# big-nacho/patolette

Measured on AMD Instinct MI355X. Metric: Mpixels/sec quantized (256-color ICtCp + KMeans) at 1 GPU; palette ΔE vs ref, higher is better.
Workload: dtype f64

## Files before the change

patolette_amd/csrc/devutil.h:

```cpp
#pragma once

#include <hip/hip_runtime.h>
#include <stdint.h>

namespace pamd {

constexpr int kWave = 64;

struct BinK {
    double M0, M1;
};

__host__ __device__ inline BinK make_bink(int E, int P) {
    int B = 51 - P;
    if (B > 40) B = 40;
    if (B < 8) B = 8;
    BinK k;
    k.M0 = ldexp(1.5, 52 + E - B);
    k.M1 = ldexp(1.5, 52 + E - 2 * B);
    return k;
}

__device__ __forceinline__ void bin_add(double v, const BinK k, double &a0, double &a1) {
    double v0 = (v + k.M0) - k.M0;
    double r = v - v0;
    double v1 = (r + k.M1) - k.M1;
    a0 += v0;
    a1 += v1;
}
__device__ __forceinline__ void bin_split(double v, const BinK k, double &v0, double &v1) {
    v0 = (v + k.M0) - k.M0;
    double r = v - v0;
    v1 = (r + k.M1) - k.M1;
}

__device__ __forceinline__ double wave_sum(double v) {
#pragma unroll
    for (int o = 32; o > 0; o >>= 1) v += __shfl_down(v, o, 64);
    return v;
}
template <int CTRL, int ROW_MASK>
__device__ __forceinline__ double dpp_add_f64(const double v) {
    const int lo = __double2loint(v), hi = __double2hiint(v);
    const int tlo = __builtin_amdgcn_update_dpp(0, lo, CTRL, ROW_MASK, 0xf, true);
    const int thi = __builtin_amdgcn_update_dpp(0, hi, CTRL, ROW_MASK, 0xf, true);
    return v + __hiloint2double(thi, tlo);
}
__device__ __forceinline__ double wave_sum_dpp63(double v) {
    v = dpp_add_f64<0x111, 0xf>(v);
    v = dpp_add_f64<0x112, 0xf>(v);
    v = dpp_add_f64<0x114, 0xf>(v);
    v = dpp_add_f64<0x118, 0xf>(v);
    v = dpp_add_f64<0x142, 0xa>(v);
    v = dpp_add_f64<0x143, 0xc>(v);
    return v;
}
__device__ __forceinline__ unsigned wave_sum_u32(unsigned v) {
#pragma unroll
    for (int o = 32; o > 0; o >>= 1) v += __shfl_down(v, o, 64);
    return v;
}

__device__ __forceinline__ unsigned wave_scan_incl_u32(unsigned v) {
    v += (unsigned)__builtin_amdgcn_update_dpp(0, (int)v, 0x111, 0xf, 0xf, true);
    v += (unsigned)__builtin_amdgcn_update_dpp(0, (int)v, 0x112, 0xf, 0xf, true);
    v += (unsigned)__builtin_amdgcn_update_dpp(0, (int)v, 0x114, 0xf, 0xf, true);
    v += (unsigned)__builtin_amdgcn_update_dpp(0, (int)v, 0x118, 0xf, 0xf, true);
    v += (unsigned)__builtin_amdgcn_update_dpp(0, (int)v, 0x142, 0xa, 0xf, true);
    v += (unsigned)__builtin_amdgcn_update_dpp(0, (int)v, 0x143, 0xc, 0xf, true);
    return v;
}

template <int NV>
__device__ __forceinline__ void block_sum(double (&v)[NV], double *smem) {
    const int lane = threadIdx.x & 63, wid = threadIdx.x >> 6, nw = blockDim.x >> 6;
#pragma unroll
    for (int i = 0; i < NV; i++) v[i] = wave_sum(v[i]);
    if (lane == 0) {
#pragma unroll
        for (int i = 0; i < NV; i++) smem[wid * NV + i] = v[i];
    }
    __syncthreads();
    if (threadIdx.x == 0) {
        for (int w = 1; w < nw; w++) {
#pragma unroll
            for (int i = 0; i < NV; i++) v[i] += smem[w * NV + i];
        }
    }
    __syncthreads();
}

__host__ __device__ inline unsigned long long f64_key(double d) {
    union { double f; unsigned long long u; } c;
    c.f = d;
    return (c.u & 0x8000000000000000ULL) ? ~c.u : (c.u | 0x8000000000000000ULL);
}
__host__ __device__ inline double key_f64(unsigned long long k) {
    union { double f; unsigned long long u; } c;
    c.u = (k & 0x8000000000000000ULL) ? (k & 0x7FFFFFFFFFFFFFFFULL) : ~k;
    return c.f;
}

__host__ __device__ inline unsigned long long splitmix64(unsigned long long x) {
    x += 0x9E3779B97F4A7C15ULL;
    unsigned long long z = x;
    z = (z ^ (z >> 30)) * 0xBF58476D1CE4E5B9ULL;
    z = (z ^ (z >> 27)) * 0x94D049BB133111EBULL;
    return z ^ (z >> 31);
}
__host__ __device__ inline double u01(unsigned long long seed, unsigned long long i) {
    return (double)(splitmix64((seed << 32) + i) >> 11) * 0x1.0p-53;
}

}
```

patolette_amd/csrc/pipeline.hip:

```cpp
#include <algorithm>
#include <functional>
#include <chrono>
#include <cmath>
#include <atomic>
#include <memory>
#include <mutex>
#include <thread>
#include <future>

#include "color_device.h"
#include "common.h"
#include "host_math.h"
#include "kmeans.h"
#include "map.h"
#include "saliency.h"
#include "quant.h"
#include "rgba.h"
#include "compact.h"

namespace pamd {

void launch_convert(int which, const double *src, double *dst, size_t n, ConvertStats *stats, hipStream_t s, BinK sumk = BinK{0.0, 0.0},
                    BinK momk = BinK{0.0, 0.0}, size_t begin = 0, size_t end = ~(size_t)0, bool init_stats = true);
void launch_convert_rows(int which, const double *rows, double *dst, size_t n, ConvertStats *stats, hipStream_t s,
                         BinK sumk = BinK{0.0, 0.0}, BinK momk = BinK{0.0, 0.0}, size_t begin = 0, size_t end = ~(size_t)0,
                         bool init_stats = true);
void launch_convert_u8(int which, const unsigned char *pixels, int channels, double *dst, size_t n, ConvertStats *stats,
                       hipStream_t s, BinK sumk = BinK{0.0, 0.0}, BinK momk = BinK{0.0, 0.0}, size_t begin = 0, size_t end = ~(size_t)0,
                       bool init_stats = true);
void launch_reconstruct(const void *map, int map_elem, size_t n, const unsigned char *pal_u8, int k, unsigned char *out,
                        hipStream_t s);
void launch_weight_stats(const double *w, size_t n, ConvertStats *stats, hipStream_t s);
void launch_pow(const double *x, double y, double *out, size_t n, hipStream_t s);
void launch_fill_image(double *d, size_t n, uint64_t seed, hipStream_t s);
void launch_fill_weights(double *d, size_t n, uint64_t seed, hipStream_t s);

KernelTimer &ktimer() { static thread_local KernelTimer *t = new KernelTimer; return *t; }

std::atomic<int> g_debug_ws{getenv("PAMD_DEBUG_WORKSPACE") ? atoi(getenv("PAMD_DEBUG_WORKSPACE")) & (kWsPoison | kWsCount | kWsLog) : 0};
std::atomic<unsigned long long> g_late_growths{0};
WsStreams &ws_streams() { static thread_local WsStreams w; return w; }
void ws_growth(size_t bytes, const char *file, int line) {
    const int dbg = g_debug_ws.load(std::memory_order_relaxed);
    if (!(dbg & (kWsCount | kWsLog))) return;
    bool queued = false;
    for (const hipStream_t *sp : ws_streams().s)
        if (sp && *sp && hipStreamQuery(*sp) == hipErrorNotReady) queued = true;
    if (!queued) return;
    g_late_growths.fetch_add(1);
    if (dbg & kWsLog) fprintf(stderr, "patolette_amd: workspace growth to %zu bytes while work is queued (%s:%d)\n", bytes, file, line);
}
void ws_poison_dev(void *p, size_t bytes) {
    if (!bytes) return;
    HIP_CHECK(hipMemsetAsync(p, 0xFF, bytes, nullptr));
    HIP_CHECK(hipStreamSynchronize(nullptr));
}
void ws_poison_dev_rows(void *p, size_t pitch, size_t width, size_t rows) {
    if (!width || !rows) return;
    HIP_CHECK(hipMemset2DAsync(p, pitch, 0xFF, width, rows, nullptr));
    HIP_CHECK(hipStreamSynchronize(nullptr));
}
int KernelTimer::id_of(const char *name) {
    for (size_t i = 0; i < names.size(); i++) if (names[i] == name) return (int)i;
    names.emplace_back(name); total_ms.push_back(0); total_bytes.push_back(0); launches.push_back(0);
    return (int)names.size() - 1;
}
hipEvent_t KernelTimer::get_event() {
    if (!pool.empty()) { hipEvent_t e = pool.back(); pool.pop_back(); return e; }
    hipEvent_t e; HIP_CHECK(hipEventCreate(&e)); return e;
}
void KernelTimer::begin(int id, hipStream_t s, double bytes, const double *src) {
    Rec r; r.id = id; r.bytes = bytes; r.src = src; r.a = get_event(); r.b = get_event();
    HIP_CHECK(hipEventRecord(r.a, s));
    pending.push_back(r);
}
void KernelTimer::end(hipStream_t s) { HIP_CHECK(hipEventRecord(pending.back().b, s)); }
void KernelTimer::collect() {
    for (auto &r : pending) {
        float ms = 0;
        if (hipEventSynchronize(r.b) == hipSuccess && hipEventElapsedTime(&ms, r.a, r.b) == hipSuccess && !(r.src && *r.src == 0.0)) {
            total_ms[r.id] += ms; total_bytes[r.id] += r.src ? r.bytes * *r.src : r.bytes; launches[r.id] += 1;
        }
        pool.push_back(r.a); pool.push_back(r.b);
    }
    pending.clear();
}
void KernelTimer::reset() { collect(); names.clear(); total_ms.clear(); total_bytes.clear(); launches.clear(); }

__global__ __launch_bounds__(256) void k_gq_prepare(Tile *tA, int ntA, Tile *tP, int ntP, unsigned long long N, int *round_nodes, int *node_tile0,
                                                    double *hist, unsigned long long nhist, unsigned long long *hsize, unsigned int *hcount) {
    const unsigned long long stride = (unsigned long long)gridDim.x * blockDim.x, t0 = (unsigned long long)blockIdx.x * blockDim.x + threadIdx.x;
    for (unsigned long long i = t0; i < (unsigned long long)ntA; i += stride) {
        const unsigned long long o = i * (unsigned long long)kTileA;
        tA[i] = Tile{o, (unsigned)(N - o < (unsigned long long)kTileA ? N - o : (unsigned long long)kTileA), 0u};
    }
    for (unsigned long long i = t0; i < (unsigned long long)ntP; i += stride) {
        const unsigned long long o = i * (unsigned long long)kTileP;
        tP[i] = Tile{o, (unsigned)(N - o < (unsigned long long)kTileP ? N - o : (unsigned long long)kTileP), 0u};
    }
    for (unsigned long long i = t0; i < nhist; i += stride) hist[i] = 0.0;
    for (unsigned long long i = t0; i < (unsigned long long)kBuckets; i += stride) { hsize[i] = 0ULL; hcount[i] = 0u; }
    if (t0 == 0) { round_nodes[0] = 0; node_tile0[0] = 0; node_tile0[1] = ntP; }
}

__global__ void k_put_nodes(NodeDev *table, const NodeIn *stage, const int *ids, int n) {
    int i = blockIdx.x * blockDim.x + threadIdx.x;
    if (i >= n) return;
    const NodeIn in = stage[i];
    NodeDev &d = table[ids[i]];
    d.begin = in.begin; d.n = in.n; d.gn = in.gn; d.buf = in.buf; d.slot = in.slot; d.child0 = in.child0; d.nchild = in.nchild;
    for (int j = 0; j < 3; j++) { d.axis[j] = in.axis[j]; d.mean[j] = in.mean[j]; }
    d.sw = in.sw; d.klin = in.klin; d.kquad = in.kquad;
    node_reset_outputs(d);
    d.split = in.split; d.psplit = -1;
}
__global__ void k_put_node1(NodeDev *table, const int id, const NodeIn in) {
    NodeDev &d = table[id];
    d.begin = in.begin; d.n = in.n; d.gn = in.gn; d.buf = in.buf; d.slot = in.slot; d.child0 = in.child0; d.nchild = in.nchild;
    for (int j = 0; j < 3; j++) { d.axis[j] = in.axis[j]; d.mean[j] = in.mean[j]; }
    d.sw = in.sw; d.klin = in.klin; d.kquad = in.kquad;
    node_reset_outputs(d);
    d.split = in.split; d.psplit = -1;
}
__global__ void k_get_nodes(const NodeDev *table, NodeOut *stage, const int *ids, int n) {
    int i = blockIdx.x * blockDim.x + threadIdx.x;
    if (i >= n) return;
    const NodeDev &d = table[ids[i]];
    NodeOut o;
    o.begin = d.begin; o.n = d.n; o.gn = d.gn; o.buf = d.buf; o.degenerate = d.degenerate; o.split = d.split; o.psplit = d.psplit;
    o.sw = d.sw;
    for (int j = 0; j < 3; j++) o.mean[j] = d.mean[j];
    for (int q = 0; q < 7; q++) {
        double s0 = 0, s1 = 0;
        for (int k = 0; k < kSlots; k++) { s0 += d.acc[k][q][0]; s1 += d.acc[k][q][1]; }
        o.acc[q][0] = s0; o.acc[q][1] = s1;
    }
    stage[i] = o;
}

struct RoundSetup {
    const NodeIn *recs; const int *ids; const int *tA0; const int *tP0;
    int nr, ntA, ntP;
    Tile *tilesA, *tilesP;
    double *hist; size_t nhist;
    unsigned long long *hsize; unsigned int *hcount; size_t nbk;
};
__device__ __forceinline__ int node_of_tile(const int *t0, int nr, int t) {
    int lo = 0, hi = nr;
    while (hi - lo > 1) { const int mid = (lo + hi) >> 1; if (t0[mid] <= t) lo = mid; else hi = mid; }
    return lo;
}
__global__ __launch_bounds__(256) void k_round_setup(NodeDev *table, RoundSetup a) {
    const size_t tid = (size_t)blockIdx.x * blockDim.x + threadIdx.x, stride = (size_t)gridDim.x * blockDim.x;
    for (size_t i = tid; i < (size_t)a.nr; i += stride) {
        const NodeIn in = a.recs[i];
        NodeDev &d = table[a.ids[i]];
        d.begin = in.begin; d.n = in.n; d.gn = in.gn; d.buf = in.buf; d.slot = in.slot; d.child0 = in.child0; d.nchild = in.nchild;
        for (int j = 0; j < 3; j++) { d.axis[j] = in.axis[j]; d.mean[j] = in.mean[j]; }
        d.sw = in.sw; d.klin = in.klin; d.kquad = in.kquad;
    }
    for (size_t i = tid; i < (size_t)a.nr * kNodeResetElems; i += stride)
        node_reset_element(table[a.ids[i / kNodeResetElems]], (int)(i % kNodeResetElems));
    for (size_t t = tid; t < (size_t)a.ntA; t += stride) {
        const int r = node_of_tile(a.tA0, a.nr, (int)t);
        const unsigned long long o = (unsigned long long)((int)t - a.tA0[r]) * kTileA, n = a.recs[r].n;
        a.tilesA[t] = Tile{a.recs[r].begin + o, (unsigned)(n - o < (unsigned long long)kTileA ? n - o : kTileA), (unsigned)a.ids[r]};
    }
    for (size_t t = tid; t < (size_t)a.ntP; t += stride) {
        const int r = node_of_tile(a.tP0, a.nr, (int)t);
        const unsigned long long o = (unsigned long long)((int)t - a.tP0[r]) * kTileP, n = a.recs[r].n;
        a.tilesP[t] = Tile{a.recs[r].begin + o, (unsigned)(n - o < (unsigned long long)kTileP ? n - o : kTileP), (unsigned)a.ids[r]};
    }
    for (size_t i = tid; i < a.nhist; i += stride) a.hist[i] = 0.0;
    for (size_t i = tid; i < a.nbk; i += stride) { a.hsize[i] = 0ULL; a.hcount[i] = 0u; }
}


struct GqOut { int kbase, error, pad[2]; int cuts[16]; unsigned long long ticks[8]; };

constexpr int kLqDevMaxK = 256;
constexpr int kLqNodeCap = 16 * kLqDevMaxK + 256;
constexpr int kLqRoundCap = 512;
constexpr int kLqMaxRounds = 96;

struct LqRec {
    double val;
    int left;
    int kn;
};
struct LqCen { double mean[3]; double gn; };
struct LqHead {
    int done, error, rounds, nnodes, neval, pad;
    unsigned long long split_evals, split_px;
    double tau;
    double round_px[kLqMaxRounds], round_nr[kLqMaxRounds];
};
struct LqCtl {
    LqHead h;
    int K, M, nleaves, pad;
    int ncids[2];
    RoundDyn dyn;
    int leaves[kLqNodeCap];
    int round_ids[kLqRoundCap];
    int cids[2][2 * kLqRoundCap];
    int tA0[kLqRoundCap + 1], tP0[kLqRoundCap + 1];
    int nparent[kLqNodeCap];
    double np[kLqNodeCap];
    LqRec nrec[kLqNodeCap];
    LqCen ncen[kLqNodeCap];
};
template <> struct WsPoison<LqCtl> {
    static void dev(LqCtl *p, size_t a, size_t b) {
        for (size_t i = a; i < b; i++) {
            char *c = reinterpret_cast<char *>(p + i);
            ws_poison_dev(c + offsetof(LqCtl, h) + offsetof(LqHead, tau), sizeof(double) * (1 + 2 * kLqMaxRounds));
            ws_poison_dev(c + offsetof(LqCtl, np), sizeof(LqCtl::np));
            ws_poison_dev_rows(c + offsetof(LqCtl, nrec), sizeof(LqRec), sizeof(double), kLqNodeCap);
            ws_poison_dev(c + offsetof(LqCtl, ncen), sizeof(LqCtl::ncen));
        }
    }
    static void host(LqCtl *, size_t, size_t) {}
};

template <int CTRL, int ROW_MASK>
__device__ __forceinline__ double dpp_max_f64(const double v) {
    const int lo = __double2loint(v), hi = __double2hiint(v);
    const int tlo = __builtin_amdgcn_update_dpp(lo, lo, CTRL, ROW_MASK, 0xf, false);
    const int thi = __builtin_amdgcn_update_dpp(hi, hi, CTRL, ROW_MASK, 0xf, false);
    return fmax(v, __hiloint2double(thi, tlo));
}

__global__ __launch_bounds__(256) void k_lq_children(NodeDev *nodes, LqCtl *c, const int call, int init_kbase,
                                                     const int init_first, int init_nnodes, const int init_K, const GqOut *gq) {
    const bool init = init_kbase > 0;
    if (!init && c->h.done) return;
    if (init && gq) { init_kbase = gq->kbase; init_nnodes = init_first + init_kbase; }
    const int ncids = init ? init_kbase : c->ncids[call & 1];
    const int wave = (int)blockIdx.x * 4 + (int)(threadIdx.x >> 6), lane = threadIdx.x & 63;
    if (init && blockIdx.x == 0 && threadIdx.x == 0) {
        c->K = init_K; c->M = init_K - init_kbase; c->nleaves = 0; c->ncids[0] = init_kbase; c->dyn = RoundDyn{0, 0, 0, 0};
        c->h.done = 0; c->h.error = 0; c->h.rounds = 0; c->h.nnodes = init_nnodes; c->h.neval = 0; c->h.split_evals = 0ULL; c->h.split_px = 0ULL;
        c->h.tau = 0.0;
        for (int r = 0; r < kLqMaxRounds; r++) { c->h.round_px[r] = 0.0; c->h.round_nr[r] = 0.0; }
        if (gq && gq->error) { c->h.done = 1; c->h.error = 3; c->ncids[0] = 0; }
        for (int i = 0; i < init_first; i++) { c->nrec[i] = LqRec{0.0, -1, 1}; c->np[i] = 0.0; c->nparent[i] = -1; }
    }
    if (init && gq && gq->error) return;
    if (wave >= ncids) return;
    const int id = init ? init_first + wave : c->cids[call & 1][wave];
    if (init && lane == 0) c->cids[0][wave] = id;
    NodeDev &d = nodes[id];
    const double *acc = &d.acc[0][0][0];
    double sum = 0;
    if (lane < 14) {
        double v[kSlots];
#pragma unroll
        for (int k = 0; k < kSlots; k++) v[k] = acc[k * 14 + lane];
#pragma unroll
        for (int k = 0; k < kSlots; k++) sum += v[k];
    }
    const double pair = sum + __shfl_down(sum, 1, 64);
    double cov[7];
#pragma unroll
    for (int q = 0; q < 7; q++)
        cov[q] = __hiloint2double(__builtin_amdgcn_readlane(__double2hiint(pair), 2 * q), __builtin_amdgcn_readlane(__double2loint(pair), 2 * q));
    if (lane != 0) return;
    double ub = cov[6];
    const bool single = d.gn <= 1ULL;
    const double sw = d.sw;
    if (single || !(sw > 0)) ub = 0;
    else {
        double c6[6];
        for (int q = 0; q < 6; q++) c6[q] = cov[q] / sw;
        const double b = hm::lambda_max_bound(c6) * sw * (1.0 + 1e-9) + 1e-9 * cov[6];
        if (b == b && b < ub) ub = b;
    }
    for (int q = 0; q < 6; q++) d.cov6[q] = cov[q];
    d.dist = cov[6]; d.ub = ub; d.axis_state = 0;
    c->nrec[id] = LqRec{single ? 0.0 : ub, -1, single ? 1 : 0};
    c->nparent[id] = init ? -1 : c->round_ids[wave >> 1];
    c->ncen[id] = LqCen{{d.mean[0], d.mean[1], d.mean[2]}, (double)d.gn};
    c->leaves[(init ? 0 : c->nleaves) + wave] = id;
}

__device__ __forceinline__ int block_excl_scan_256(const int v, int *sw , int &total) {
    const int lane = threadIdx.x & 63, wid = threadIdx.x >> 6;
    const int inc = (int)wave_scan_incl_u32((unsigned)v);
    __syncthreads();
    if (lane == 63) sw[wid] = inc;
    __syncthreads();
    int base = 0;
    for (int w = 0; w < wid; w++) base += sw[w];
    total = sw[0] + sw[1] + sw[2] + sw[3];
    return base + inc - v;
}

__device__ __forceinline__ unsigned long long lq_key(const double p) { return p > 0.0 ? (unsigned long long)__double_as_longlong(p) : 0ULL; }

constexpr double kSpecBeta = 0.25;

__global__ __launch_bounds__(256) void k_lq_select(NodeDev *nodes, LqCtl *c, const int call, const int e_lin, const int e_quad) {
    if (c->h.done) return;
    const int tid = threadIdx.x, lane = tid & 63;
    const int cur = call & 1, nxt = cur ^ 1;
    const int ncids = c->ncids[cur];
    if (blockIdx.x > 0) {
        const int w = ((int)blockIdx.x - 1) * 4 + (tid >> 6);
        if (w >= ncids) return;
        NodeDev &d = nodes[c->cids[cur][w]];
        if (d.gn <= 1ULL || !(d.sw > 0)) { if (lane == 0) d.axis_state = d.gn <= 1ULL ? 0 : -1; return; }
        double c6[6];
        for (int q = 0; q < 6; q++) c6[q] = d.cov6[q] / d.sw;
        double a[9] = {c6[0], c6[1], c6[2], c6[1], c6[3], c6[4], c6[2], c6[4], c6[5]};
        double wv[3];
        const int info = hm::eigen_sym3(a, wv);
        if (lane == 0) {
            if (info != 0) d.axis_state = -1;
            else { d.axis[0] = a[6]; d.axis[1] = a[7]; d.axis[2] = a[8]; d.axis_state = 1; }
        }
        return;
    }
    __shared__ int sw[5];
    __shared__ unsigned int hist[256];
    __shared__ unsigned long long s_prefix, s_px;
    __shared__ int s_need, s_neval, s_first;
    __shared__ double s_umax[4];
    const int M = c->M;
    const int nn = c->h.nnodes;
    const int nr_prev = c->dyn.nr;
    int evald = 0;
    for (int i = tid; i < nr_prev; i += 256) {
        const int id = c->round_ids[i];
        const NodeDev &d = nodes[id];
        if (d.axis_state < 0) { c->nrec[id] = LqRec{0.0, -1, 1}; c->np[id] = 0.0; continue; }
        const int l = d.child0;
        const double b = d.dist - (nodes[l].dist + nodes[l + 1].dist);
        const int par = c->nparent[id];
        const double pp = par < 0 ? INFINITY : c->np[par];
        c->nrec[id].val = b; c->nrec[id].kn = 1;
        c->np[id] = b < pp ? b : pp;
        evald++;
    }
    if (tid == 0) { s_neval = 0; s_px = 0ULL; }
    __syncthreads();
    if (evald) atomicAdd(&s_neval, evald);
    __syncthreads();
    const int neval = c->h.neval + s_neval;
    double tau = 0.0;
    if (neval >= M && M > 0) {
        unsigned long long prefix = 0ULL;
        int need = M;
        for (int pass = 0; pass < 3; pass++) {
            const int shift = 56 - 8 * pass;
            hist[tid] = 0u;
            __syncthreads();
            for (int i = tid; i < nn; i += 256) {
                const LqRec r = c->nrec[i];
                if (r.kn && r.left >= 0) {
                    const unsigned long long k = lq_key(c->np[i]);
                    if (pass == 0 || (k >> (shift + 8)) == (prefix >> (shift + 8))) atomicAdd(&hist[(k >> shift) & 255ULL], 1u);
                }
            }
            __syncthreads();
            {
                const int mine = (int)hist[255 - tid];
                int total;
                const int excl = block_excl_scan_256(mine, sw, total);
                if (tid == 0) s_first = 256;
                __syncthreads();
                if (excl + mine >= need && tid <= 254) atomicMin(&s_first, tid);
                __syncthreads();
                const int f = s_first;
                if (f < 256) { if (tid == f) { s_need = need - excl; s_prefix = prefix | ((unsigned long long)(255 - f) << shift); } }
                else if (tid == 254) { s_need = need - (excl + mine); s_prefix = prefix; }
            }
            __syncthreads();
            need = s_need; prefix = s_prefix;
        }
        tau = __longlong_as_double((long long)prefix);
    }
    const double thr = fmax(kDelta, tau * (1.0 - 1e-9));
    const int nleaves = c->nleaves + ncids;
    auto leaf_prio = [&](const int id) -> double {
        const LqRec r = c->nrec[id];
        const int par = c->nparent[id];
        if (r.kn || (par >= 0 && nodes[par].axis_state < 0)) return -1.0;
        const double pp = par < 0 ? INFINITY : c->np[par];
        return r.val < pp ? r.val : pp;
    };
    double thr2 = thr;
    if (c->h.rounds < 48) {
        double u = -1.0;
        for (int i = tid; i < nleaves; i += 256) { const double pr = leaf_prio(c->leaves[i]); u = pr > u ? pr : u; }
#pragma unroll
        for (int o = 32; o > 0; o >>= 1) { const double v = __shfl_xor(u, o, 64); u = v > u ? v : u; }
        __syncthreads();
        if (lane == 0) s_umax[tid >> 6] = u;
        __syncthreads();
        u = fmax(fmax(s_umax[0], s_umax[1]), fmax(s_umax[2], s_umax[3]));
        if (kSpecBeta * u > thr2) thr2 = kSpecBeta * u;
    }
    int nkeep = 0, nr = 0;
    for (int base = 0; base < nleaves; base += 256) {
        const int i = base + tid;
        int id = -1, sel = 0, keep = 0;
        if (i < nleaves) {
            id = c->leaves[i];
            const double pr = leaf_prio(id);
            sel = pr >= thr2 ? 1 : 0;
            keep = (!sel && pr >= thr) ? 1 : 0;
        }
        int tsel, tkeep;
        const int psel = block_excl_scan_256(sel, sw, tsel);
        if (nr + tsel > kLqRoundCap && sel && nr + psel >= kLqRoundCap) { sel = 0; keep = 1; }
        const int pkeep = block_excl_scan_256(keep, sw, tkeep);
        if (sel) c->round_ids[nr + psel] = id;
        __syncthreads();
        if (keep) c->leaves[nkeep + pkeep] = id;
        nr = min(nr + tsel, kLqRoundCap);
        nkeep += tkeep;
        __syncthreads();
    }
    if (nr == 0) {
        if (tid == 0) { c->h.done = 1; c->h.neval = neval; c->h.tau = tau; c->nleaves = 0; c->ncids[nxt] = 0; c->dyn = RoundDyn{0, 0, 0, 0}; }
        return;
    }
    if (nn + 2 * nr > kLqNodeCap) {
        if (tid == 0) { c->h.done = 1; c->h.error = 2; c->dyn = RoundDyn{0, 0, 0, 0}; }
        return;
    }
    int runA = 0, runP = 0;
    for (int base = 0; base < nr; base += 256) {
        const int r = base + tid;
        int ta = 0, tp = 0;
        unsigned long long n = 0ULL;
        if (r < nr) {
            const int id = c->round_ids[r];
            NodeDev &d = nodes[id];
            d.slot = r; d.child0 = nn + 2 * r; d.nchild = 2;
            int P = 1;
            while ((1ULL << P) < (d.gn > 1ULL ? d.gn : 2ULL)) P++;
            d.klin = make_bink(e_lin, P); d.kquad = make_bink(e_quad, P);
            c->nrec[id].left = nn + 2 * r;
            c->cids[nxt][2 * r] = nn + 2 * r; c->cids[nxt][2 * r + 1] = nn + 2 * r + 1;
            n = d.n;
            ta = (int)((n + kTileA - 1) / kTileA); tp = (int)((n + kTileP - 1) / kTileP);
        }
        int totA, totP;
        const int pa = block_excl_scan_256(ta, sw, totA);
        const int pp = block_excl_scan_256(tp, sw, totP);
        if (r < nr) { c->tA0[r] = runA + pa; c->tP0[r] = runP + pp; }
        runA += totA; runP += totP;
        for (int o = 32; o > 0; o >>= 1) n += __shfl_xor(n, o, 64);
        if (lane == 0 && n) atomicAdd(&s_px, n);
    }
    __syncthreads();
    if (tid == 0) {
        const int round = c->h.rounds;
        const unsigned long long rpx = s_px;
        c->tA0[nr] = runA; c->tP0[nr] = runP;
        c->nleaves = nkeep; c->ncids[nxt] = 2 * nr;
        c->dyn = RoundDyn{nr, runA, runP, 0};
        c->h.nnodes = nn + 2 * nr; c->h.neval = neval; c->h.tau = tau;
        c->h.split_evals += (unsigned long long)nr; c->h.split_px += rpx; c->h.rounds = round + 1;
        if (round < kLqMaxRounds) { c->h.round_px[round] = (double)rpx; c->h.round_nr[round] = (double)nr; }
    }
}

__global__ __launch_bounds__(256) void k_lq_export(const LqCtl *c, LqHead *head, LqRec *rec, LqCen *cen) {
    const int nn = c->h.nnodes;
    const int t = blockIdx.x * blockDim.x + threadIdx.x, stride = gridDim.x * blockDim.x;
    for (int i = t; i < nn; i += stride) { rec[i] = c->nrec[i]; cen[i] = c->ncen[i]; }
    const double *src = reinterpret_cast<const double *>(&c->h);
    double *dst = reinterpret_cast<double *>(head);
    for (int i = t; i < (int)(sizeof(LqHead) / sizeof(double)); i += stride) dst[i] = src[i];
}

struct LqCommit { int row, node, new_row, left; };
__global__ void k_lq_trace(const NodeDev *nodes, const LqCommit *commits, int n, patolette_amd__SplitRecord *out) {
    const int t = blockIdx.x * blockDim.x + threadIdx.x;
    if (t >= n) return;
    const LqCommit cm = commits[t];
    const NodeDev &h = nodes[cm.node], &hl = nodes[cm.left], &hr = nodes[cm.left + 1];
    patolette_amd__SplitRecord tr;
    tr.row = cm.row; tr.new_row = cm.new_row;
    tr.split = hl.psplit < 0 ? -1 : (hl.psplit & 0xffff); tr.degenerate = hl.psplit < 0 ? 0 : (hl.psplit >> 16) & 1;
    tr.n = h.gn; tr.n_left = hl.gn; tr.n_right = hr.gn; tr.sw = h.sw;
    for (int j = 0; j < 3; j++) tr.axis[j] = h.axis[j];
    for (int q = 0; q < 6; q++) tr.cov6[q] = h.cov6[q] / h.sw;
    tr.dist = h.dist; tr.dist_left = hl.dist; tr.dist_right = hr.dist; tr.benefit = h.dist - (hl.dist + hr.dist);
    out[t] = tr;
}

__global__ __launch_bounds__(256) void k_round_setup_dyn(NodeDev *table, const LqCtl *c, Tile *tilesA, Tile *tilesP, double *hist,
                                                         unsigned long long *hsize, unsigned int *hcount, const size_t lqs) {
    const int nr = c->dyn.nr;
    if (nr == 0) return;
    const int ntA = c->dyn.ntA, ntP = c->dyn.ntP;
    const size_t tid = (size_t)blockIdx.x * blockDim.x + threadIdx.x, stride = (size_t)gridDim.x * blockDim.x;
    for (size_t i = tid; i < (size_t)nr * kNodeResetElems; i += stride)
        node_reset_element(table[c->round_ids[i / kNodeResetElems]], (int)(i % kNodeResetElems));
    for (size_t t = tid; t < (size_t)ntA; t += stride) {
        const int r = node_of_tile(c->tA0, nr, (int)t);
        const NodeDev &d = table[c->round_ids[r]];
        const unsigned long long o = (unsigned long long)((int)t - c->tA0[r]) * kTileA, n = d.n;
        tilesA[t] = Tile{d.begin + o, (unsigned)(n - o < (unsigned long long)kTileA ? n - o : kTileA), (unsigned)c->round_ids[r]};
    }
    for (size_t t = tid; t < (size_t)ntP; t += stride) {
        const int r = node_of_tile(c->tP0, nr, (int)t);
        const NodeDev &d = table[c->round_ids[r]];
        const unsigned long long o = (unsigned long long)((int)t - c->tP0[r]) * kTileP, n = d.n;
        tilesP[t] = Tile{d.begin + o, (unsigned)(n - o < (unsigned long long)kTileP ? n - o : kTileP), (unsigned)c->round_ids[r]};
    }
    for (size_t i = tid; i < lqs * (size_t)nr; i += stride) hist[i] = 0.0;
    for (size_t i = tid; i < (size_t)nr * kBuckets; i += stride) { hsize[i] = 0ULL; hcount[i] = 0u; }
}

struct GqTab {
    unsigned long long w0[kBuckets + 1];
    double t[10][kBuckets + 9];
    __device__ double distortion(int a, int b) const {
        if (w0[a] == w0[b]) return 0;
        const double q0 = t[0][b] - t[0][a], q1 = t[1][b] - t[1][a], q2 = t[2][b] - t[2][a];
        return t[3][b] - t[3][a] - (q0 * q0 + q1 * q1 + q2 * q2) / (double)(w0[b] - w0[a]);
    }
    __device__ double vcov(int a, int b, int r, int s) const {
        if (w0[a] == w0[b]) return 0;
        const double cnt = (double)(w0[b] - w0[a]);
        const int rs = 4 + s * (s + 1) / 2 + r;
        return (t[rs][b] - t[rs][a]) / cnt - (t[r][b] - t[r][a]) * (t[s][b] - t[s][a]) / (cnt * cnt);
    }
    __device__ bool axis(int a, int b, double ax[3]) const {
        double m[9] = {0, 0, 0, 0, 0, 0, 0, 0, 0};
        for (int s = 0; s < 3; s++) for (int r = 0; r <= s; r++) m[s * 3 + r] = vcov(a, b, r, s);
        m[0 * 3 + 2] = m[2 * 3 + 0]; m[0 * 3 + 1] = m[1 * 3 + 0]; m[1 * 3 + 2] = m[2 * 3 + 1];
        double w[3];
        if (hm::eigen_sym3(m, w) != 0) return false;
        ax[0] = m[6]; ax[1] = m[7]; ax[2] = m[8];
        return true;
    }
    __device__ static double norm3(const double a[3]) { double s = 0; for (int i = 0; i < 3; i++) s += a[i] * a[i]; return sqrt(s); }
    __device__ double bias(int a, int b, const double ax[3]) const {
        double ca[3];
        if (!axis(a, b, ca)) return -1;
        const double norms = norm3(ax) * norm3(ca);
        if (norms < 1e-16) return 0;
        const double dot = (ca[0] * ax[0] + ca[1] * ax[1] + ca[2] * ax[2]);
        return fmin(1.0, fabs(dot / norms));
    }
};

__device__ __forceinline__ void gq_dp_entry(const GqTab &c, const double *Ep, const int k, const int n, const int lane, double &e_out, int &cut_out) {
    double best = INFINITY; int bt = -1;
    for (int t = n - 2 - lane; t >= k - 1; t -= 64) {
        const double v = Ep[t] + c.distortion(t, n);
        if (v < best) { best = v; bt = t; }
    }
#pragma unroll
    for (int o = 32; o > 0; o >>= 1) {
        const double v2 = __shfl_down(best, o, 64); const int t2 = __shfl_down(bt, o, 64);
        if (t2 >= 0 && (bt < 0 || v2 < best || (v2 == best && t2 > bt))) { best = v2; bt = t2; }
    }
    double e = Ep[n - 1]; int cut = n - 1;
    if (bt >= 0 && best < e) { e = best; cut = bt; }
    e_out = e; cut_out = cut;
}

__global__ __launch_bounds__(1024) void k_gq_control(const double *__restrict__ hist, const unsigned int *__restrict__ hcount, GqDpDev *g,
                                                     const int palette_size, const int weighted, NodeDev *nodes, const int base0,
                                                     unsigned char *lut, GqOut *out, GqOut *out_host) {
    __shared__ GqTab c;
    __shared__ double E[2][kBuckets + 1];
    __shared__ int s_q[16], s_nq, s_stop, s_err, s_top;
    __shared__ double s_ax[3], s_cd[16], s_cb[16];
    __shared__ unsigned char s_lut[kBuckets];
    __shared__ double s_part[kGqMaxK][4][2];
    __shared__ unsigned long long s_cnt[kGqMaxK];
    const int tid = threadIdx.x, lane = tid & 63, wv = tid >> 6;
    __shared__ unsigned long long s_ticks[8];
    if (tid == 0) { for (int i = 0; i < 8; i++) s_ticks[i] = 0; s_ticks[0] = wall_clock64(); }
    for (int i = tid; i < 10 * kBuckets; i += 1024) {
        const int hq = i / kBuckets, b = i - hq * kBuckets;
        c.t[hq][b + 1] = hist[(size_t)(hq * 2 + 0) * kBuckets + b] + hist[(size_t)(hq * 2 + 1) * kBuckets + b];
    }
    for (int b = tid; b < kBuckets; b += 1024) c.w0[b + 1] = hcount[b];
    if (tid < 10) c.t[tid][0] = 0;
    if (tid == 10) c.w0[0] = 0;
    __syncthreads();
    if (tid == 0) s_ticks[5] = wall_clock64();
    if (wv < 10) {
        double *t = c.t[wv];
        double v[8];
#pragma unroll
        for (int u = 0; u < 8; u++) v[u] = t[1 + lane * 8 + u];
        double carry = 0, cin = 0;
        for (int l = 0; l < 64; l++) {
            double a = carry;
#pragma unroll
            for (int u = 0; u < 8; u++) a = v[u] + a;
            cin = lane == l ? carry : cin;
            carry = __hiloint2double(__builtin_amdgcn_readlane(__double2hiint(a), l), __builtin_amdgcn_readlane(__double2loint(a), l));
        }
        double a = cin;
#pragma unroll
        for (int u = 0; u < 8; u++) { a = v[u] + a; t[1 + lane * 8 + u] = a; }
    }
    if (wv == 10) {
        unsigned long long v[8], run = 0;
#pragma unroll
        for (int u = 0; u < 8; u++) { run += c.w0[1 + lane * 8 + u]; v[u] = run; }
        unsigned long long inc = run;
#pragma unroll
        for (int o = 1; o < 64; o <<= 1) { const unsigned long long t = __shfl_up(inc, o, 64); if (lane >= o) inc += t; }
        const unsigned long long before = inc - run;
#pragma unroll
        for (int u = 0; u < 8; u++) c.w0[1 + lane * 8 + u] = before + v[u];
    }
    __syncthreads();
    if (tid == 0) s_ticks[1] = wall_clock64();
    for (int i = tid; i < (kGqMaxK + 1) * (kBuckets + 1); i += 1024) { const int r = i / (kBuckets + 1), n = i - r * (kBuckets + 1); g->cut[r][n] = r == n ? r : 0; }
    for (int i = tid; i <= kBuckets; i += 1024) E[1][i] = i >= 1 ? c.distortion(0, i) : 0.0;
    if (tid == 0) {
        double ax[3] = {0, 0, 0};
        s_err = c.axis(0, kBuckets, ax) ? 0 : 1;
        s_ax[0] = ax[0]; s_ax[1] = ax[1]; s_ax[2] = ax[2];
        s_q[0] = 0; s_q[1] = kBuckets; s_nq = 2; s_stop = 0;
    }
    __syncthreads();
    const int kmax = palette_size < kGqMaxK ? palette_size : kGqMaxK;
    if (tid == 0) s_ticks[2] = wall_clock64();
    for (int k = 2; k <= kmax && !s_err; k++) {
        const int cells = s_nq - 1;
        if (lane == 0 && wv < cells) {
            const double ax[3] = {s_ax[0], s_ax[1], s_ax[2]};
            s_cd[wv] = c.distortion(s_q[wv], s_q[wv + 1]);
            if (cells == 1) {
                const double norms = GqTab::norm3(ax) * GqTab::norm3(ax);
                s_cb[wv] = norms < 1e-16 ? 0.0 : fmin(1.0, fabs((ax[0] * ax[0] + ax[1] * ax[1] + ax[2] * ax[2]) / norms));
            } else s_cb[wv] = c.bias(s_q[wv], s_q[wv + 1], ax);
        }
        __syncthreads();
        if (tid == 0) {
            double distortion = 0;
            for (int j = 0; j < cells; j++) distortion += s_cd[j];
            int stop = 0;
            if (distortion < 1e-16) stop = 1;
            else {
                double bias = 0;
                for (int i = 0; i < cells; i++) {
                    const double cd = s_cd[i], cb = s_cb[i];
                    if (cb < 0) { stop = 1; break; }
                    if (cb < 0.9) continue;
                    bias += (cd / distortion) * cb;
                }
                if (!stop) stop = bias < 0.1 ? 1 : 0;
            }
            s_stop = stop;
        }
        __syncthreads();
        if (s_stop) break;
        if (k > 2) {
            const int kk = k - 1;
            const double *Ep = E[(kk - 1) & 1];
            double *En = E[kk & 1];
            for (int n = wv; n <= kBuckets; n += 16) {
                if (n < kk + 1) { if (lane == 0) En[n] = Ep[n]; continue; }
                double e; int cut;
                gq_dp_entry(c, Ep, kk, n, lane, e, cut);
                if (lane == 0) { En[n] = e; g->cut[kk][n] = cut; }
            }
            __syncthreads();
        }
        if (wv == 0) {
            double e; int cut;
            gq_dp_entry(c, E[(k - 1) & 1], k, kBuckets, lane, e, cut);
            if (lane == 0) s_top = cut;
        }
        __syncthreads();
        if (tid == 0) {
            int t = s_top;
            s_q[k - 1] = t;
            for (int j = k - 2; j >= 1; j--) { t = g->cut[j + 1][t]; s_q[j] = t; }
            s_q[0] = 0; s_q[k] = kBuckets; s_nq = k + 1;
        }
        __syncthreads();
    }
    const int kbase = s_nq - 1;
    if (tid == 0) s_ticks[3] = wall_clock64();
    for (int b = tid; b < kBuckets; b += 1024) {
        int j = 0;
        while (j < kbase - 1 && !(b + 1 <= s_q[j + 1])) j++;
        s_lut[b] = (unsigned char)j;
        lut[b] = (unsigned char)j;
    }
    __syncthreads();
    const int nq = weighted ? 4 : 3;
    if (wv < 2 * nq) {
        const int q = wv >> 1, part = wv & 1, qi = weighted ? 10 + q : q;
        const double *h = hist + (size_t)(qi * 2 + part) * kBuckets + lane * 8;
        double v[8];
#pragma unroll
        for (int u = 0; u < 8; u++) v[u] = h[u];
        for (int j = 0; j < kbase; j++) {
            double a = 0;
#pragma unroll
            for (int u = 0; u < 8; u++) a += s_lut[lane * 8 + u] == j ? v[u] : 0.0;
#pragma unroll
            for (int o = 32; o > 0; o >>= 1) a += __shfl_xor(a, o, 64);
            if (lane == 0) s_part[j][q][part] = a;
        }
    } else if (wv == 8) {
        unsigned long long v[8];
#pragma unroll
        for (int u = 0; u < 8; u++) v[u] = hcount[lane * 8 + u];
        for (int j = 0; j < kbase; j++) {
            unsigned long long a = 0;
#pragma unroll
            for (int u = 0; u < 8; u++) a += s_lut[lane * 8 + u] == j ? v[u] : 0ULL;
#pragma unroll
            for (int o = 32; o > 0; o >>= 1) a += __shfl_xor(a, o, 64);
            if (lane == 0) s_cnt[j] = a;
        }
    }
    __syncthreads();
    if (tid < kbase) {
        const int j = tid;
        unsigned long long pos = 0;
        for (int i = 0; i < j; i++) pos += s_cnt[i];
        const unsigned long long cnt = s_cnt[j];
        NodeDev &ch = nodes[base0 + j];
        ch.begin = pos; ch.n = cnt; ch.gn = cnt; ch.buf = 1; ch.slot = -1; ch.child0 = -1; ch.nchild = 0;
        const double sw = weighted ? (s_part[j][3][0] + s_part[j][3][1]) : (double)cnt;
        const double inv = 1 / sw;
        for (int q = 0; q < 3; q++) { ch.axis[q] = 0; ch.mean[q] = (s_part[j][q][0] + s_part[j][q][1]) * inv; }
        ch.sw = sw; ch.klin = nodes[0].klin; ch.kquad = nodes[0].kquad;
        node_reset_outputs(ch);
        ch.split = -1; ch.psplit = -1;
    }
    if (tid == 64) {
        NodeDev &root = nodes[0];
        root.child0 = base0; root.nchild = kbase;
        root.split = kbase == 2 ? s_q[1] - 1 : -1;
        GqOut o;
        o.kbase = kbase; o.error = s_err; o.pad[0] = o.pad[1] = 0;
        for (int j = 0; j < 16; j++) o.cuts[j] = j <= kbase ? s_q[j] : 0;
        for (int j = 0; j < 8; j++) o.ticks[j] = s_ticks[j];
        o.ticks[4] = wall_clock64();
        *out = o;
        *out_host = o;
    }
}

__global__ void k_eigen_batch(const double *a9, size_t count, double *w3, double *z9, int *info) {
    const size_t i = (size_t)blockIdx.x * blockDim.x + threadIdx.x;
    if (i >= count) return;
    double a[9], w[3];
    for (int j = 0; j < 9; j++) a[j] = a9[i * 9 + j];
    info[i] = hm::eigen_sym3(a, w);
    for (int j = 0; j < 3; j++) w3[i * 3 + j] = w[j];
    for (int j = 0; j < 9; j++) z9[i * 9 + j] = a[j];
}

__global__ void k_shard_pack_keys(const NodeDev *table, const int *ids, int n, int rank, int size, unsigned long long *buf) {
    const int i = blockIdx.x * blockDim.x + threadIdx.x;
    if (i >= n) return;
    const NodeDev &d = table[ids[i]];
    unsigned long long a = ~0ULL, b = 0ULL;
    for (int k = 0; k < kSlots; k++) { a = d.minkey[k] < a ? d.minkey[k] : a; b = d.maxkey[k] > b ? d.maxkey[k] : b; }
    for (int r = 0; r < size; r++) {
        unsigned long long *row = buf + ((size_t)r * n + i) * 3;
        row[0] = r == rank ? a : 0ULL; row[1] = r == rank ? b : 0ULL; row[2] = r == rank ? d.n : 0ULL;
    }
}
__global__ void k_shard_unpack_keys(NodeDev *table, const int *ids, int n, int rank, int size, const unsigned long long *buf) {
    const int i = blockIdx.x * blockDim.x + threadIdx.x;
    if (i >= n) return;
    NodeDev &d = table[ids[i]];
    unsigned long long a = ~0ULL, b = 0ULL, before = 0ULL;
    for (int r = 0; r < size; r++) {
        const unsigned long long *row = buf + ((size_t)r * n + i) * 3;
        a = row[0] < a ? row[0] : a; b = row[1] > b ? row[1] : b;
        if (r < rank) before += row[2];
    }
    for (int k = 0; k < kSlots; k++) { d.minkey[k] = ~0ULL; d.maxkey[k] = 0ULL; }
    d.minkey[0] = a; d.maxkey[0] = b; d.gslot0 = before;
}
__global__ void k_shard_pack_acc(const NodeDev *table, const int *ids, int n, double *buf) {
    const int i = blockIdx.x * blockDim.x + threadIdx.x;
    if (i >= n) return;
    const NodeDev &d = table[ids[i]];
    for (int q = 0; q < 7; q++) {
        double s0 = 0, s1 = 0;
        for (int k = 0; k < kSlots; k++) { s0 += d.acc[k][q][0]; s1 += d.acc[k][q][1]; }
        buf[(size_t)i * 14 + 2 * q] = s0; buf[(size_t)i * 14 + 2 * q + 1] = s1;
    }
}
__global__ void k_shard_unpack_acc(NodeDev *table, const int *ids, int n, const double *buf) {
    const int i = blockIdx.x * blockDim.x + threadIdx.x;
    if (i >= n) return;
    NodeDev &d = table[ids[i]];
    for (int q = 0; q < 7; q++) {
        for (int k = 1; k < kSlots; k++) { d.acc[k][q][0] = 0; d.acc[k][q][1] = 0; }
        d.acc[0][q][0] = buf[(size_t)i * 14 + 2 * q]; d.acc[0][q][1] = buf[(size_t)i * 14 + 2 * q + 1];
    }
}
__global__ void k_shard_children_local(NodeDev *table, const int *round_nodes, int nround) {
    const int i = blockIdx.x * blockDim.x + threadIdx.x;
    if (i >= nround) return;
    const NodeDev &nd = table[round_nodes[i]];
    for (int k = 0; k < nd.nchild; k++) {
        NodeDev &ch = table[nd.child0 + k];
        ch.begin = nd.cbegin[k]; ch.n = nd.cbegin[k + 1] - nd.cbegin[k];
    }
}

struct Bounds {
    double cmax, range, wmax; int e_lin, e_quad; double lo[3], hi[3];
    bool have_sum = false; double sum[3] = {0, 0, 0};
// ... 201 lines not shown
}
static const int *shard_upload_ids(Engine &E, const std::vector<int> &ids) {
    E.shard_ids.reserve(ids.size());
    HIP_CHECK(hipStreamSynchronize(E.stream));
    HIP_CHECK(hipMemcpy(E.shard_ids.p, ids.data(), ids.size() * sizeof(int), hipMemcpyHostToDevice));
    return E.shard_ids.p;
}

static double now_ms() {
    return std::chrono::duration<double, std::milli>(std::chrono::steady_clock::now().time_since_epoch()).count();
}

struct HNode {
    unsigned long long begin = 0, n = 0;
    unsigned long long gn = 0;
    int buf = 0;
    double sw = 0, mean[3] = {0, 0, 0}, cov6[6] = {0, 0, 0, 0, 0, 0}, dist = 0;
    int left = -1, right = -1;
    int psplit = -1;
    bool split_done = false, nosplit = false;
    int axis_state = 0;
    double axis[3] = {0, 0, 0};
    double ub = 0;
};

static void build_tiles(const std::vector<int> &round, const std::vector<HNode> &hn, int tile, std::vector<Tile> &out,
                        std::vector<int> *tile0) {
    out.clear();
    if (tile0) tile0->clear();
    for (size_t r = 0; r < round.size(); r++) {
        const HNode &nd = hn[round[r]];
        if (tile0) tile0->push_back((int)out.size());
        for (unsigned long long o = 0; o < nd.n; o += (unsigned long long)tile) {
            Tile t;
            t.start = nd.begin + o;
            t.count = (unsigned)std::min<unsigned long long>((unsigned long long)tile, nd.n - o);
            t.node = (unsigned)round[r];
            out.push_back(t);
        }
    }
    if (tile0) tile0->push_back((int)out.size());
}

static NodeIn make_nodedev(const HNode &h, const Bounds &b) {
    NodeIn d;
    std::memset(&d, 0, sizeof d);
    d.begin = h.begin; d.n = h.n; d.gn = h.gn; d.buf = h.buf; d.slot = -1; d.child0 = -1; d.nchild = 0; d.split = -1;
    for (int j = 0; j < 3; j++) d.mean[j] = h.mean[j];
    d.sw = h.sw;
    int P = 1;
    while ((1ULL << P) < (h.gn > 1 ? h.gn : 2)) P++;
    d.klin = make_bink(b.e_lin, P);
    d.kquad = make_bink(b.e_quad, P);
    return d;
}

static void upload_tiles(Engine &E, const std::vector<Tile> &t, DevBuf<Tile> &dst, PinBuf<Tile> &stage) {
    if (t.empty()) return;
    dst.reserve(t.size());
    stage.reserve(t.size());
    std::memcpy(stage.p, t.data(), t.size() * sizeof(Tile));
    HIP_CHECK(hipMemcpyAsync(dst.p, stage.p, t.size() * sizeof(Tile), hipMemcpyHostToDevice, E.stream));
}
static void upload_ints(Engine &E, const std::vector<int> &v, DevBuf<int> &dst, PinBuf<int> &stage) {
    if (v.empty()) return;
    dst.reserve(v.size());
    stage.reserve(v.size());
    std::memcpy(stage.p, v.data(), v.size() * sizeof(int));
    HIP_CHECK(hipMemcpyAsync(dst.p, stage.p, v.size() * sizeof(int), hipMemcpyHostToDevice, E.stream));
}

static void put_nodes(Engine &E, const std::vector<int> &ids, const std::vector<NodeIn> &recs) {
    const int n = (int)ids.size();
    if (!n) return;
    if (n == 1) {
        hipLaunchKernelGGL(k_put_node1, 1, 1, 0, E.stream, E.nodes.p, ids[0], recs[0]);
        HIP_CHECK(hipGetLastError());
        return;
    }
    E.stage_in.reserve(n); E.ids.reserve(n); E.h_stage_in.reserve(n); E.h_ids.reserve(n);
    std::memcpy(E.h_stage_in.p, recs.data(), n * sizeof(NodeIn));
    std::memcpy(E.h_ids.p, ids.data(), n * sizeof(int));
    HIP_CHECK(hipMemcpyAsync(E.stage_in.p, E.h_stage_in.p, n * sizeof(NodeIn), hipMemcpyHostToDevice, E.stream));
    HIP_CHECK(hipMemcpyAsync(E.ids.p, E.h_ids.p, n * sizeof(int), hipMemcpyHostToDevice, E.stream));
    hipLaunchKernelGGL(k_put_nodes, (n + 63) / 64, 64, 0, E.stream, E.nodes.p, E.stage_in.p, E.ids.p, n);
    HIP_CHECK(hipGetLastError());
}

static void get_nodes(Engine &E, const std::vector<int> &ids, std::vector<NodeOut> &recs) {
    const int n = (int)ids.size();
    recs.resize(n);
    if (!n) return;
    E.stage_out.reserve(n); E.ids.reserve(n); E.h_stage_out.reserve(n); E.h_ids_get.reserve(n);
    std::memcpy(E.h_ids_get.p, ids.data(), n * sizeof(int));
    HIP_CHECK(hipMemcpyAsync(E.ids.p, E.h_ids_get.p, n * sizeof(int), hipMemcpyHostToDevice, E.stream));
    hipLaunchKernelGGL(k_get_nodes, (n + 63) / 64, 64, 0, E.stream, E.nodes.p, E.stage_out.p, E.ids.p, n);
    HIP_CHECK(hipGetLastError());
    HIP_CHECK(hipMemcpyAsync(E.h_stage_out.p, E.stage_out.p, n * sizeof(NodeOut), hipMemcpyDeviceToHost, E.stream));
    E.sync();
    std::memcpy(recs.data(), E.h_stage_out.p, n * sizeof(NodeOut));
}

static void get_nodes_dev(Engine &E, const int *d_ids, int n, std::vector<NodeOut> &recs) {
    recs.resize(n);
    if (!n) return;
    E.h_stage_out.reserve(n);
    hipLaunchKernelGGL(k_get_nodes, (n + 63) / 64, 64, 0, E.stream, E.nodes.p, E.h_stage_out.p, d_ids, n);
    HIP_CHECK(hipGetLastError());
    E.sync();
    std::memcpy(recs.data(), E.h_stage_out.p, n * sizeof(NodeOut));
}

static void absorb_moments(HNode &h, const NodeOut &d) {
    for (int q = 0; q < 6; q++) h.cov6[q] = d.acc[q][0] + d.acc[q][1];
    h.dist = d.acc[6][0] + d.acc[6][1];
}

static bool node_axis(const HNode &h, double axis[3]) {
    if (h.axis_state != 0) {
        for (int j = 0; j < 3; j++) axis[j] = h.axis[j];
        return h.axis_state > 0;
    }
    double c6[6];
    for (int q = 0; q < 6; q++) c6[q] = h.cov6[q] / h.sw;
    return hm::principal_axis(c6, axis);
}

static void leaf_bound(HNode &h) {
    h.ub = h.dist;
    h.axis_state = 0;
    if (h.gn <= 1 || !(h.sw > 0)) { h.ub = 0; return; }
    double c6[6];
    for (int q = 0; q < 6; q++) c6[q] = h.cov6[q] / h.sw;
    double a[9] = {c6[0], c6[1], c6[2], c6[1], c6[3], c6[4], c6[2], c6[4], c6[5]};
    double w[3];
    if (hm::eigen_sym3(a, w) != 0) { h.axis_state = -1; return; }
    h.axis[0] = a[6]; h.axis[1] = a[7]; h.axis[2] = a[8]; h.axis_state = 1;
    const double b = w[2] * h.sw * (1.0 + 1e-9) + 1e-9 * h.dist;
    if (b == b && b < h.ub) h.ub = b;
}

static void gq_prepare(Engine &E, size_t N, bool weighted) {
    hipStream_t s = E.stream;
    const size_t planes = weighted ? 4 : 3;
    E.bufA.reserve(planes * N + 64); E.bufB.reserve(planes * N + 64); E.bkt.reserve(N);
    const int ntA = (int)ceil_div(N, (size_t)kTileA), ntP = (int)ceil_div(N, (size_t)kTileP);
    E.tilesA.reserve(ntA); E.tilesP.reserve(ntP);
    E.h_round.reserve(kBuckets);
    E.round_nodes.reserve(1); E.node_tile0.reserve(2);
    E.tilecnt.reserve((size_t)ntP * kMaxChildren); E.tileoff.reserve((size_t)ntP * kMaxChildren);
    const size_t hs = hist_slot_doubles();
    E.hist.reserve(hs); E.hsize.reserve(kBuckets); E.hcount.reserve(kBuckets); E.lut.reserve(kBuckets);
    hipLaunchKernelGGL(k_gq_prepare, 64, 256, 0, s, E.tilesA.p, ntA, E.tilesP.p, ntP, (unsigned long long)N, E.round_nodes.p, E.node_tile0.p,
                       E.hist.p, (unsigned long long)hs, E.hsize.p, E.hcount.p);
    HIP_CHECK(hipGetLastError());
    E.prep_N = N; E.prep_planes = planes;
}



struct LqReplay { std::vector<int> result; std::vector<LqCommit> commits; bool stopped_early = false; };
static bool lq_replay_plain(const LqRec *rec, int kbase, int first_base, size_t K, LqReplay &out) {
    std::vector<int> &result = out.result;
    result.assign(K, -1);
    for (int j = 0; j < kbase; j++) result[j] = first_base + j;
    size_t count = (size_t)kbase;
    std::vector<double> fval(K, 0.0);
    std::vector<char> fkn(K, 0);
    for (size_t j = 0; j < count; j++) { fval[j] = rec[result[j]].val; fkn[j] = (char)rec[result[j]].kn; }
    const int fault = g_debug_fault.load(std::memory_order_relaxed);
    while (count < K) {
        int best = -1; double bv = 0, mu = -1;
        for (size_t j = 0; j < count; j++) {
            if (fkn[j]) { if (best < 0 || fval[j] > bv) { bv = fval[j]; best = (int)j; } }
            else if (fval[j] > mu) mu = fval[j];
        }
        if (mu < 0 || (best >= 0 && bv > mu)) {
            if (fault == 2) {
                int second = -1; double sv = -1;
                for (size_t j = 0; j < count; j++) if ((int)j != best && fkn[j] && fval[j] > sv) { sv = fval[j]; second = (int)j; }
                if (second >= 0 && sv >= kDelta && sv < bv) { best = second; bv = sv; }
            }
            if (!(bv >= kDelta)) { out.stopped_early = true; break; }
            const int id = result[best], l = rec[id].left;
            out.commits.push_back(LqCommit{best, id, (int)count, l});
            result[count] = l; result[best] = l + 1;
            fval[count] = rec[l].val; fkn[count] = (char)rec[l].kn;
            fval[best] = rec[l + 1].val; fkn[best] = (char)rec[l + 1].kn;
            count++;
            continue;
        }
        if (std::max(best >= 0 ? bv : 0.0, mu) < kDelta) { out.stopped_early = true; break; }
        return false;
    }
    result.resize(count);
    return true;
}

static bool lq_replay(const LqRec *rec, int kbase, int first_base, size_t K, LqReplay &out) {
    std::vector<int> &result = out.result;
    result.assign(K, -1);
    for (int j = 0; j < kbase; j++) result[j] = first_base + j;
    size_t count = (size_t)kbase;
    constexpr size_t B = 16;
    const size_t nb = (K + B - 1) / B;
    std::vector<double> fval(nb * B, 0.0);
    std::vector<char> fkn(nb * B, 0);
    std::vector<double> bbv(nb, 0.0), bmu(nb, -1.0);
    std::vector<int> bbest(nb, -1);
    auto rescan = [&](const size_t b) {
        int best = -1; double bv = 0, mu = -1;
        const size_t lo = b * B, hi = std::min(count, lo + B);
        for (size_t j = lo; j < hi; j++) {
            if (fkn[j]) { if (best < 0 || fval[j] > bv) { bv = fval[j]; best = (int)j; } }
            else if (fval[j] > mu) mu = fval[j];
        }
        bbest[b] = best; bbv[b] = bv; bmu[b] = mu;
    };
    for (size_t j = 0; j < count; j++) { fval[j] = rec[result[j]].val; fkn[j] = (char)rec[result[j]].kn; }
    for (size_t b = 0; b < nb; b++) rescan(b);
    const int fault = g_debug_fault.load(std::memory_order_relaxed);
    while (count < K) {
        int best = -1; double bv = 0, mu = -1;
        const size_t nbu = (count + B - 1) / B;
        for (size_t b = 0; b < nbu; b++) {
            if (bbest[b] >= 0 && (best < 0 || bbv[b] > bv)) { bv = bbv[b]; best = bbest[b]; }
            if (bmu[b] > mu) mu = bmu[b];
        }
        if (mu < 0 || (best >= 0 && bv > mu)) {
            if (fault == 2) {
                int second = -1; double sv = -1;
                for (size_t j = 0; j < count; j++) if ((int)j != best && fkn[j] && fval[j] > sv) { sv = fval[j]; second = (int)j; }
                if (second >= 0 && sv >= kDelta && sv < bv) { best = second; bv = sv; }
            }
            if (!(bv >= kDelta)) { out.stopped_early = true; break; }
            const int id = result[best], l = rec[id].left;
            out.commits.push_back(LqCommit{best, id, (int)count, l});
            result[count] = l; result[best] = l + 1;
            fval[count] = rec[l].val; fkn[count] = (char)rec[l].kn;
            fval[best] = rec[l + 1].val; fkn[best] = (char)rec[l + 1].kn;
            count++;
            rescan((size_t)best / B);
            if ((count - 1) / B != (size_t)best / B) rescan((count - 1) / B);
            continue;
        }
        if (std::max(best >= 0 ? bv : 0.0, mu) < kDelta) { out.stopped_early = true; break; }
        return false;
    }
    result.resize(count);
    return true;
}

std::atomic<int> g_lq_device{getenv("PAMD_LQ_DEVICE") ? atoi(getenv("PAMD_LQ_DEVICE")) : 2};
std::atomic<int> g_gq_device{getenv("PAMD_GQ_DEVICE") ? atoi(getenv("PAMD_GQ_DEVICE")) : 1};
constexpr size_t kLqDeviceAutoPixels = (size_t)40 << 20;

static bool lq_device_eligible(const Engine &E, size_t N, size_t K, bool verbose, bool allow_device) {
    const int lq_mode = g_lq_device.load(std::memory_order_relaxed);
    return allow_device && (lq_mode == 1 || (lq_mode == 2 && N < kLqDeviceAutoPixels)) && !E.shard && !verbose && K <= (size_t)kLqDevMaxK;
}

static void ws_prepare(Engine &E, size_t N, size_t K, bool weighted, bool verbose) {
    const size_t planes = weighted ? 4 : 3;
    const bool lq_dev = lq_device_eligible(E, N, K, verbose, true);
    const size_t slack = lq_dev ? (size_t)kLqRoundCap : 0, ntA = ceil_div(N, (size_t)kTileA) + slack, ntP = ceil_div(N, (size_t)kTileP) + slack;
    const size_t tables = lq_dev ? (size_t)kLqRoundCap * kBuckets : (size_t)kBuckets;
    E.cvt.reserve(planes * N); E.cstats.reserve(1);
    E.bufA.reserve(planes * N + 64); E.bufB.reserve(planes * N + 64); E.bkt.reserve(N);
    E.tilesA.reserve(ntA); E.tilesP.reserve(ntP);
    E.tilecnt.reserve(ntP * kMaxChildren); E.tileoff.reserve(ntP * kMaxChildren);
    E.round_nodes.reserve(1); E.node_tile0.reserve(2); E.h_round.reserve(kBuckets);
    E.hist.reserve(std::max(hist_slot_doubles(), lq_dev ? (size_t)kNQ_LQ * 2 * kBuckets * kLqRoundCap : 0));
    E.hsize.reserve(tables); E.hcount.reserve(tables); E.lut.reserve(tables);
    E.nodes.reserve(std::max<size_t>(4 * K + 64, lq_dev ? (size_t)kLqNodeCap : 0));
    E.h_dbl.reserve(16 * kBuckets * 2 + 64);
    E.gq.reserve(1); E.gqout.reserve(1); E.h_gqout.reserve(1); E.h_gq.reserve(1);
    const size_t nput = kGqMaxK + 1;
    E.stage_in.reserve(nput); E.stage_out.reserve(nput); E.ids.reserve(nput); E.h_stage_in.reserve(nput); E.h_stage_out.reserve(nput);
    E.h_ids.reserve(nput); E.h_ids_get.reserve(nput);
    E.h_cent.reserve(3 * K);
    if (lq_dev) { E.lqctl.reserve(1); E.h_lqhead.reserve(1); E.h_lqrec.reserve(kLqNodeCap); E.h_lqcen.reserve(kLqNodeCap); }
}

static int lq_device_loop(Engine &E, size_t N, size_t K, bool weighted, bool inv_sums, const Bounds &bnd, const QuantBuffers &qlq, int kbase,
                          int first_base, int nnodes, std::vector<double> &centers, size_t &len, unsigned long long *max_members) {
    hipStream_t s = E.stream;
    const size_t lqs = (size_t)kNQ_LQ * 2 * kBuckets;
    const int ntA_ub = (int)ceil_div(N, (size_t)kTileA) + kLqRoundCap, ntP_ub = (int)ceil_div(N, (size_t)kTileP) + kLqRoundCap;
    E.lqctl.reserve(1); E.h_lqhead.reserve(1); E.h_lqrec.reserve(kLqNodeCap); E.h_lqcen.reserve(kLqNodeCap);
    E.hist.reserve(std::max(hist_slot_doubles(), lqs * kLqRoundCap)); E.hsize.reserve((size_t)kLqRoundCap * kBuckets);
    E.hcount.reserve((size_t)kLqRoundCap * kBuckets); E.lut.reserve((size_t)kLqRoundCap * kBuckets);
    E.tilesA.reserve(ntA_ub); E.tilesP.reserve(ntP_ub);
    E.tilecnt.reserve((size_t)ntP_ub * kMaxChildren); E.tileoff.reserve((size_t)ntP_ub * kMaxChildren);
    LqCtl *c = E.lqctl.p;
    LqHead *head = E.h_lqhead.p;
    for (int r = 0; r < kLqMaxRounds; r++) { head->round_px[r] = 0.0; head->round_nr[r] = 0.0; }
    const RoundDyn *dyn = &c->dyn;
    const int *d_round = c->round_ids, *d_tP0 = c->tP0;
    int call = 0;
    const GqOut *gq = kbase < 0 ? (const GqOut *)E.gqout.p : nullptr;
    const int kb_ub = kbase < 0 ? kGqMaxK : kbase;
    auto control = [&]() {
        const bool first = call == 0;
        {
            KTIME("k_lq_children", s, 0.0);
            if (first) hipLaunchKernelGGL(k_lq_children, (kb_ub + 3) / 4, 256, 0, s, E.nodes.p, c, call, kb_ub, first_base, nnodes, (int)K, gq);
            else hipLaunchKernelGGL(k_lq_children, 2 * kLqRoundCap / 4, 256, 0, s, E.nodes.p, c, call, 0, 0, 0, 0, (const GqOut *)nullptr);
        }
        KTIME("k_lq_select", s, 0.0);
        hipLaunchKernelGGL(k_lq_select, 1 + (first ? (kb_ub + 3) / 4 : 2 * kLqRoundCap / 4), 256, 0, s, E.nodes.p, c, call, bnd.e_lin, bnd.e_quad);
        HIP_CHECK(hipGetLastError());
        call++;
    };
    int enq = 0;
    auto round = [&]() {
        if (enq >= kLqMaxRounds) throw HipError("patolette_amd: split loop exceeded its round limit");
        const double *px_src = &head->round_px[enq], *nr_src = &head->round_nr[enq];
        const bool rev = enq % 2 == 1;
        static const bool setup_kernel = getenv("PAMD_LQ_SETUP_KERNEL") && atoi(getenv("PAMD_LQ_SETUP_KERNEL")) != 0;
        if (setup_kernel) {
            hipLaunchKernelGGL(k_round_setup_dyn, 1024, 256, 0, s, E.nodes.p, (const LqCtl *)c, E.tilesA.p, E.tilesP.p, E.hist.p, E.hsize.p, E.hcount.p, lqs);
            HIP_CHECK(hipGetLastError());
            launch_minmax(qlq, E.tilesA.p, ntA_ub, 0, E.nodes.p, s, rev, dyn, px_src);
        } else {
            const RoundLists rl{c->round_ids, c->tA0, c->tP0, E.tilesA.p, E.tilesP.p, E.hist.p, lqs, E.hsize.p, E.hcount.p};
            launch_minmax(qlq, E.tilesA.p, ntA_ub, 0, E.nodes.p, s, rev, dyn, px_src, &rl);
        }
        launch_hist(qlq, false, E.tilesA.p, ntA_ub, 0, E.nodes.p, E.hist.p, E.hsize.p, E.hcount.p, s, !rev, false, dyn, px_src);
        launch_cut(weighted, E.nodes.p, d_round, kLqRoundCap, E.hist.p, E.hsize.p, E.hcount.p, E.lut.p, s, dyn, nr_src);
        launch_partition(qlq, E.tilesP.p, ntP_ub, 0, d_round, d_tP0, kLqRoundCap, E.nodes.p, E.lut.p, E.tilecnt.p, E.tileoff.p, true, s, inv_sums, rev, dyn, px_src);
        enq++;
        control();
    };
    control();
    int want = (E.lq_hint_N == N && E.lq_hint_K == K && E.lq_hint_rounds > 0) ? E.lq_hint_rounds : 9;
    const bool fault_full = g_debug_fault.load(std::memory_order_relaxed) == 4;
    if (fault_full) want = 3;
    for (;;) {
        while (enq < want) round();
        hipLaunchKernelGGL(k_lq_export, 16, 256, 0, s, (const LqCtl *)c, head, E.h_lqrec.p, E.h_lqcen.p);
        HIP_CHECK(hipGetLastError());
        E.sync();
        if (fault_full) return -2;
        if (head->done) break;
        want = enq + 2;
    }
    if (head->error == 2) return -2;
    if (head->error == 3) return -1;
    if (kbase < 0) kbase = E.h_gqout.p->kbase;
    E.lq_hint_N = N; E.lq_hint_K = K; E.lq_hint_rounds = head->rounds;
    LqReplay rp;
    const double t_rp0 = now_ms();
    E.lq_rec_local.resize((size_t)head->nnodes);
    std::memcpy(E.lq_rec_local.data(), E.h_lqrec.p, (size_t)head->nnodes * sizeof(LqRec));
    const bool replay_ok = lq_replay(E.lq_rec_local.data(), kbase, first_base, K, rp);
    const double t_rp1 = now_ms();
    static const bool replay_check = getenv("PAMD_LQ_REPLAY_CHECK") != nullptr;
    if (replay_check || !replay_ok) {
        LqReplay ref;
        const bool ref_ok = lq_replay_plain(E.lq_rec_local.data(), kbase, first_base, K, ref);
        if (ref_ok != replay_ok || ref.result != rp.result || ref.stopped_early != rp.stopped_early)
            fprintf(stderr, "patolette_amd: split loop: the two replays DISAGREE (plain %d, %zu rows; blocked %d, %zu rows), kbase %d, K %zu, nodes %d, rounds %d\n",
                    (int)ref_ok, ref.result.size(), (int)replay_ok, rp.result.size(), kbase, K, head->nnodes, head->rounds);
        else if (!replay_ok)
            fprintf(stderr, "patolette_amd: split loop: both replays blocked after %zu commits, kbase %d, K %zu, nodes %d, rounds %d, evaluated %d, tau %.17g\n",
                    rp.commits.size(), kbase, K, head->nnodes, head->rounds, head->neval, head->tau);
    }
    if (!replay_ok) throw HipError("patolette_amd: split loop: the replay met an unevaluated node");
    len = rp.result.size();
    centers.assign(3 * len, 0.0);
    unsigned long long mg = 0;
    for (size_t i = 0; i < len; i++) {
        const LqCen &cn = E.h_lqcen.p[rp.result[i]];
        for (int j = 0; j < 3; j++) centers[(size_t)j * len + i] = cn.mean[j];
        mg = std::max(mg, (unsigned long long)cn.gn);
    }
    if (max_members) *max_members = mg;
    E.stats.split_evals = (size_t)head->split_evals; E.stats.split_px = (size_t)head->split_px; E.stats.lq_rounds = (size_t)head->rounds;
    E.lq_commits.swap(rp.commits);
    E.trace.clear();
    E.trace_pending = true;
    E.trace_hdr.stopped_early = rp.stopped_early ? 1 : 0;
    static const bool lq_times = getenv("PAMD_LQ_TIMES") != nullptr;
    if (lq_times) {
        fprintf(stderr, "patolette_amd: device-driven split loop: %d rounds, %d evaluated, %zu commits, tau %.3g; host replay %.1f us\n", head->rounds, head->neval,
                E.lq_commits.size(), head->tau, 1e3 * (t_rp1 - t_rp0));
        if (gq) {
            const unsigned long long *t = E.h_gqout.p->ticks;
            fprintf(stderr, "patolette_amd: k_gq_control us: prefixes %.1f, axis %.1f, search %.1f, records %.1f\n", (t[1] - t[0]) * 0.01, (t[2] - t[1]) * 0.01,
                    (t[3] - t[2]) * 0.01, (t[4] - t[3]) * 0.01);
            fprintf(stderr, "patolette_amd: k_gq_control us: of the prefixes, staging %.1f\n", (t[5] - t[0]) * 0.01);
        }
    }
    return 0;
}

static void materialise_trace(Engine &E) {
    if (!E.trace_pending) return;
    E.trace_pending = false;
    const int n = (int)E.lq_commits.size();
    E.trace.assign(n, patolette_amd__SplitRecord{});
    if (!n) return;
    DevBuf<LqCommit> dc; DevBuf<patolette_amd__SplitRecord> dr;
    dc.reserve(n); dr.reserve(n);
    HIP_CHECK(hipMemcpyAsync(dc.p, E.lq_commits.data(), sizeof(LqCommit) * n, hipMemcpyHostToDevice, E.stream));
    hipLaunchKernelGGL(k_lq_trace, (n + 63) / 64, 64, 0, E.stream, (const NodeDev *)E.nodes.p, (const LqCommit *)dc.p, n, dr.p);
    HIP_CHECK(hipGetLastError());
    HIP_CHECK(hipMemcpyAsync(E.trace.data(), dr.p, sizeof(patolette_amd__SplitRecord) * n, hipMemcpyDeviceToHost, E.stream));
    HIP_CHECK(hipStreamSynchronize(E.stream));
}

static int quantize_clusters_run(Engine &E, size_t N, size_t K, bool weighted, const Bounds &bnd,
                                 std::vector<double> &centers, size_t &len, bool verbose, unsigned long long *max_members, bool allow_device) {
    hipStream_t s = E.stream;
    const size_t planes = weighted ? 4 : 3;
    const Shard *sh = E.shard;
    const size_t Nt = sh ? sh->total : N;
    const bool inv_sums = sh || E.invariant;
    if (E.prep_N != N || E.prep_planes != planes) gq_prepare(E, N, weighted);
    E.prep_N = 0;
    const bool dev_eligible = lq_device_eligible(E, N, K, verbose, allow_device);
    E.nodes.reserve(std::max<size_t>(4 * K + 64, dev_eligible ? (size_t)kLqNodeCap : 0));
    std::vector<HNode> hn;
    hn.reserve(4 * K + 64);
    double t0 = now_ms();

    HNode root; root.begin = 0; root.n = N; root.gn = Nt; root.buf = 0; root.sw = (double)Nt;
    E.h_dbl.reserve(16 * kBuckets * 2 + 64);
    if (bnd.have_sum) {
        const double inv = 1 / (double)Nt;
        for (int j = 0; j < 3; j++) root.mean[j] = bnd.sum[j] * inv;
    } else {
        int rootP = 1; while ((1ULL << rootP) < (Nt > 1 ? Nt : 2)) rootP++;
        E.sum6.reserve(kSum3Slots * 6);
        launch_sum3(E.cvt.p, N, make_bink(bnd.e_lin, rootP), E.sum6.p, s);
        if (sh) comm_sum_dev(E, E.sum6.p, kSum3Slots * 6, 0);
        HIP_CHECK(hipMemcpyAsync(E.h_dbl.p, E.sum6.p, kSum3Slots * 6 * sizeof(double), hipMemcpyDeviceToHost, s));
        E.sync();
        const double inv = 1 / (double)Nt;
        for (int j = 0; j < 3; j++) {
            double p0 = 0, p1 = 0;
            for (int sl = 0; sl < kSum3Slots; sl++) { p0 += E.h_dbl.p[sl * 6 + 2 * j]; p1 += E.h_dbl.p[sl * 6 + 2 * j + 1]; }
            root.mean[j] = (p0 + p1) * inv;
        }
    }
    hn.push_back(root);
    QuantBuffers qroot{{E.cvt.p, E.bufA.p}, E.bkt.p, N, weighted};
    QuantBuffers qlq{{E.bufB.p, E.bufA.p}, E.bkt.p, N, weighted};
    std::vector<int> round = {0};
    const int ntA0 = (int)ceil_div(N, (size_t)kTileA), ntP0 = (int)ceil_div(N, (size_t)kTileP);
    std::vector<NodeOut> got;
    bool mom_path = bnd.have_mom && !sh;
    if (mom_path) {
        const long double nn = (long double)Nt;
        long double s1[3], c6[6], s2d[3] = {0, 0, 0};
        for (int j = 0; j < 3; j++) s1[j] = (long double)bnd.sum2[j][0] + (long double)bnd.sum2[j][1];
        static const int ja[6] = {0, 1, 2, 1, 2, 2}, jb[6] = {0, 0, 0, 1, 1, 2};
        for (int q = 0; q < 6; q++) {
            const long double s2 = (long double)bnd.mom2[q][0] + (long double)bnd.mom2[q][1];
            if (ja[q] == jb[q]) s2d[ja[q]] = s2;
            c6[q] = s2 - s1[ja[q]] * s1[jb[q]] / nn;
        }
        const long double tr = c6[0] + c6[3] + c6[5], tr2 = s2d[0] + s2d[1] + s2d[2];
        if (!(tr > 1e-6L * tr2) || c6[0] < 0 || c6[3] < 0 || c6[5] < 0) mom_path = false;
        else {
            for (int q = 0; q < 6; q++) hn[0].cov6[q] = (double)c6[q];
            hn[0].dist = (double)tr;
        }
    }
    if (!mom_path) {
        NodeIn d = make_nodedev(hn[0], bnd);
        put_nodes(E, {0}, {d});
        launch_cov_nodes(qroot, E.cvt.p, E.tilesA.p, ntA0, N, E.nodes.p, s, true);
        if (sh) shard_exchange_acc(E, shard_upload_ids(E, {0}), 1);
        get_nodes(E, {0}, got);
        absorb_moments(hn[0], got[0]);
    }
    double axis[3];
    if (!node_axis(hn[0], axis)) return -1;
    E.trace.clear();
    E.trace_pending = false;
    E.trace_hdr = patolette_amd__SplitTrace{};
    for (int j = 0; j < 3; j++) E.trace_hdr.gq_axis[j] = axis[j];
    for (int q = 0; q < 6; q++) E.trace_hdr.gq_cov6[q] = hn[0].cov6[q] / hn[0].sw;

    {
        NodeIn d = make_nodedev(hn[0], bnd);
        for (int j = 0; j < 3; j++) d.axis[j] = axis[j];
        d.slot = 0;
        put_nodes(E, {0}, {d});
    }
    const size_t hs = hist_slot_doubles();
    launch_minmax(qroot, E.tilesA.p, ntA0, N, E.nodes.p, s, mom_path);
    if (sh) shard_exchange_keys(E, shard_upload_ids(E, {0}), 1);
    launch_hist(qroot, true, E.tilesA.p, ntA0, N, E.nodes.p, E.hist.p, E.hsize.p, E.hcount.p, s, !mom_path, Nt >= ((size_t)1 << 18));
    if (sh) { comm_sum_dev(E, E.hist.p, hs, 0); comm_sum_dev(E, E.hcount.p, kBuckets, 2); }
    const bool gq_dev = g_gq_device.load(std::memory_order_relaxed) != 0 && !sh && !verbose && K > (size_t)kGqMaxK;
    int kbase = 0;
    std::vector<int> base_ids;
    if (gq_dev) {
        E.gq.reserve(1); E.gqout.reserve(1); E.h_gqout.reserve(1);
        *E.h_gqout.p = GqOut{};
        {
            KTIME("k_gq_control", s, (double)hs * 8);
            hipLaunchKernelGGL(k_gq_control, 1, 1024, 0, s, (const double *)E.hist.p, (const unsigned int *)E.hcount.p, E.gq.p, (int)std::min<size_t>(K, (size_t)1 << 30),
                               weighted ? 1 : 0, E.nodes.p, 1, E.lut.p, E.gqout.p, E.h_gqout.p);
            HIP_CHECK(hipGetLastError());
        }
        launch_partition(qroot, E.tilesP.p, ntP0, N, E.round_nodes.p, E.node_tile0.p, 1, E.nodes.p, E.lut.p, E.tilecnt.p, E.tileoff.p, true, s, inv_sums,
                         mom_path, nullptr, nullptr, true);
        launch_cov_children(qroot, E.tilesA.p, ntA0, N, E.nodes.p, s, !mom_path, true);
        auto trace_header = [&]() {
            const GqOut &o = *E.h_gqout.p;
            E.trace_hdr.n_base = o.kbase;
            for (int j = 0; j <= o.kbase && j < 14; j++) E.trace_hdr.gq_cuts[j] = (size_t)o.cuts[j];
        };
        if (dev_eligible) {
            E.stats.ms_gq = now_ms() - t0;
            t0 = now_ms();
            const int rc = lq_device_loop(E, N, K, weighted, inv_sums, bnd, qlq, -1, 1, 0, centers, len, max_members);
            trace_header();
            E.stats.n_base_clusters = (size_t)E.h_gqout.p->kbase;
            if (rc != 0) return rc;
            E.stats.n_clusters = len;
            E.trace_hdr.n_clusters = (int32_t)len; E.trace_hdr.n_records = (int32_t)E.lq_commits.size();
            E.cluster_centers = centers;
            E.stats.ms_lq = now_ms() - t0;
            return 0;
        }
        std::vector<int> all(kGqMaxK);
        for (int j = 0; j < kGqMaxK; j++) all[j] = 1 + j;
        get_nodes(E, all, got);
        if (E.h_gqout.p->error) return -1;
        trace_header();
        kbase = E.h_gqout.p->kbase;
        for (int j = 0; j < kbase; j++) {
            HNode c; c.buf = 1; c.begin = got[j].begin; c.n = got[j].n; c.gn = got[j].gn; c.sw = got[j].sw;
            for (int q = 0; q < 3; q++) c.mean[q] = got[j].mean[q];
            absorb_moments(c, got[j]);
            leaf_bound(c);
            base_ids.push_back((int)hn.size());
            hn.push_back(c);
        }
    } else {
    const int gq_kmax = (int)std::min<size_t>(K, kGqMaxK);
    E.gq.reserve(1); E.h_gq.reserve(1);
    launch_gq_dp(E.hist.p, E.hcount.p, gq_kmax, E.gq.p, s);
    HIP_CHECK(hipMemcpyAsync(E.h_gq.p->cut, E.gq.p->cut, sizeof(E.h_gq.p->cut), hipMemcpyDeviceToHost, s));
    std::vector<double> hh(hs);
    std::vector<unsigned int> hc(kBuckets);
    HIP_CHECK(hipMemcpyAsync(E.h_dbl.p, E.hist.p, hs * sizeof(double), hipMemcpyDeviceToHost, s));
    E.h_round.reserve(kBuckets);
    HIP_CHECK(hipMemcpyAsync(E.h_round.p, E.hcount.p, kBuckets * sizeof(unsigned int), hipMemcpyDeviceToHost, s));
    E.sync();
    std::memcpy(hh.data(), E.h_dbl.p, hs * sizeof(double));
    std::memcpy(hc.data(), E.h_round.p, kBuckets * sizeof(unsigned int));
    auto H = [&](int q, int b) { return hh[(size_t)(q * 2 + 0) * kBuckets + b] + hh[(size_t)(q * 2 + 1) * kBuckets + b]; };

    auto cm = std::make_unique<hm::CellMoments>();
    std::memset(cm.get(), 0, sizeof(hm::CellMoments));
    for (int b = 0; b < kBuckets; b++) {
        cm->w0[b + 1] = hc[b];
        for (int r = 0; r < 3; r++) cm->w1[r][b + 1] = H(r, b);
        cm->w2[b + 1] = H(3, b);
        for (int q = 0; q < 6; q++) cm->wrs[q][b + 1] = H(4 + q, b);
    }
    for (int i = 1; i <= kBuckets; i++) {
        cm->w0[i] += cm->w0[i - 1]; cm->w2[i] += cm->w2[i - 1];
        for (int r = 0; r < 3; r++) cm->w1[r][i] += cm->w1[r][i - 1];
        for (int q = 0; q < 6; q++) cm->wrs[q][i] += cm->wrs[q][i - 1];
    }
    std::vector<size_t> cuts = hm::gq_principal_quantizer(K, *cm, E.h_gq.p->cut);
    if (cuts.size() < 2) return -1;
    kbase = (int)cuts.size() - 1;
    E.trace_hdr.n_base = kbase;
    for (int j = 0; j <= kbase && j < 14; j++) E.trace_hdr.gq_cuts[j] = cuts[j];

    std::vector<unsigned char> lut(kBuckets);
    for (int b = 0; b < kBuckets; b++) {
        int j = 0;
        while (j < kbase - 1 && !((size_t)(b + 1) <= cuts[j + 1])) j++;
        lut[b] = (unsigned char)j;
    }
    const bool gq_binary = kbase == 2;
    {
        unsigned long long pos = 0;
        for (int j = 0; j < kbase; j++) {
            HNode c; c.buf = 1; c.begin = pos;
            unsigned long long cnt = 0;
            double s0[4] = {0, 0, 0, 0}, s1[4] = {0, 0, 0, 0};
            for (int b = 0; b < kBuckets; b++) if (lut[b] == j) {
                cnt += hc[b];
                for (int q = 0; q < (weighted ? 4 : 3); q++) {
                    int qi = weighted ? 10 + q : q;
                    s0[q] += hh[(size_t)(qi * 2 + 0) * kBuckets + b];
                    s1[q] += hh[(size_t)(qi * 2 + 1) * kBuckets + b];
                }
            }
            c.n = cnt; c.gn = cnt;
            c.sw = weighted ? (s0[3] + s1[3]) : (double)cnt;
            const double inv = 1 / c.sw;
            for (int q = 0; q < 3; q++) c.mean[q] = (s0[q] + s1[q]) * inv;
            pos += cnt;
            base_ids.push_back((int)hn.size());
            hn.push_back(c);
        }
    }
    {
        NodeIn d = make_nodedev(hn[0], bnd);
        for (int j = 0; j < 3; j++) d.axis[j] = axis[j];
        d.slot = 0; d.child0 = base_ids[0]; d.nchild = kbase;
        if (gq_binary) d.split = (int)cuts[1] - 1;
        std::vector<int> ids = {0};
        std::vector<NodeIn> recs = {d};
        for (int id : base_ids) { ids.push_back(id); NodeIn c = make_nodedev(hn[id], bnd); c.klin = d.klin; c.kquad = d.kquad; recs.push_back(c); }
        put_nodes(E, ids, recs);
    }
    E.h_bytes.reserve(kBuckets);
    std::memcpy(E.h_bytes.p, lut.data(), kBuckets);
    HIP_CHECK(hipMemcpyAsync(E.lut.p, E.h_bytes.p, kBuckets, hipMemcpyHostToDevice, s));
    launch_partition(qroot, E.tilesP.p, ntP0, N, E.round_nodes.p, E.node_tile0.p, 1, E.nodes.p, E.lut.p, E.tilecnt.p, E.tileoff.p, gq_binary, s, inv_sums, mom_path);
    if (sh) { hipLaunchKernelGGL(k_shard_children_local, 1, 64, 0, s, E.nodes.p, E.round_nodes.p, 1); HIP_CHECK(hipGetLastError()); }
    if (!gq_binary) launch_cov_children(qroot, E.tilesA.p, ntA0, N, E.nodes.p, s, !mom_path);
    if (sh) shard_exchange_acc(E, shard_upload_ids(E, base_ids), (int)base_ids.size());
    if (dev_eligible && (size_t)kbase < K) {
        E.stats.n_base_clusters = (size_t)kbase;
        E.stats.ms_gq = now_ms() - t0;
        t0 = now_ms();
        const int rc = lq_device_loop(E, N, K, weighted, inv_sums, bnd, qlq, kbase, base_ids[0], (int)hn.size(), centers, len, max_members);
        if (rc != 0) return rc;
        E.stats.n_clusters = len;
        E.trace_hdr.n_clusters = (int32_t)len; E.trace_hdr.n_records = (int32_t)E.lq_commits.size();
        E.cluster_centers = centers;
// ... 1625 lines not shown
```

patolette_amd/csrc/quant.h:

```cpp
#pragma once

#include <atomic>

#include "common.h"
#include "devutil.h"

namespace pamd {

constexpr int kMaxChildren = 16;
constexpr int kTileA = 8192;
constexpr int kTileP = 2048;

constexpr int kNQ_LQ = 4;
constexpr int kNQ_GQ = 14;

constexpr int kSlots = 16;

struct NodeIn {
    unsigned long long begin, n, gn;
    int buf, slot, child0, nchild;
    int split;
    double axis[3], mean[3], sw;
    BinK klin, kquad;
};
struct NodeOut {
    unsigned long long begin, n, gn;
    int buf, degenerate, split, psplit;
    double sw, mean[3];
    double acc[7][2];
};

struct NodeDev {
    unsigned long long begin;
    unsigned long long n;
    unsigned long long gn;
    unsigned long long gslot0;
    int buf;
    int slot;
    int child0;
    int nchild;
    double axis[3];
    double mean[3];
    double sw;
    BinK klin, kquad;
    unsigned long long minkey[kSlots], maxkey[kSlots];
    int degenerate;
    int split;
    int psplit;
    int axis_state;
    double cov6[6], dist, ub;
    unsigned long long cbegin[kMaxChildren + 1];
    double acc[kSlots][7][2];
};

template <> struct WsPoison<NodeDev> {
    static void dev(NodeDev *p, size_t a, size_t b) {
        char *c = reinterpret_cast<char *>(p + a);
        ws_poison_dev_rows(c + offsetof(NodeDev, axis), sizeof(NodeDev), offsetof(NodeDev, klin) - offsetof(NodeDev, axis), b - a);
        ws_poison_dev_rows(c + offsetof(NodeDev, cov6), sizeof(NodeDev), offsetof(NodeDev, cbegin) - offsetof(NodeDev, cov6), b - a);
        ws_poison_dev_rows(c + offsetof(NodeDev, acc), sizeof(NodeDev), sizeof(NodeDev::acc), b - a);
    }
    static void host(NodeDev *, size_t, size_t) {}
};

__device__ __forceinline__ void node_reset_outputs(NodeDev &d) {
    for (int i = 0; i < kSlots; i++) { d.minkey[i] = ~0ULL; d.maxkey[i] = 0ULL; }
    for (int i = 0; i < kSlots; i++) for (int q = 0; q < 7; q++) { d.acc[i][q][0] = 0; d.acc[i][q][1] = 0; }
    d.degenerate = 0; d.split = -1; d.gslot0 = 0;
}
constexpr int kNodeResetElems = kSlots * 14 + 2 * kSlots;
__device__ __forceinline__ void node_reset_element(NodeDev &d, int e) {
    if (e < kSlots * 14) (&d.acc[0][0][0])[e] = 0.0;
    else if (e < kSlots * 15) d.minkey[e - kSlots * 14] = ~0ULL;
    else d.maxkey[e - kSlots * 15] = 0ULL;
    if (e == 0) { d.degenerate = 0; d.split = -1; d.gslot0 = 0; }
}
__device__ __forceinline__ void node_minmax(const NodeDev &d, double &mn, double &mx) {
    unsigned long long a = ~0ULL, b = 0ULL;
    for (int i = 0; i < kSlots; i++) { a = d.minkey[i] < a ? d.minkey[i] : a; b = d.maxkey[i] > b ? d.maxkey[i] : b; }
    mn = key_f64(a); mx = key_f64(b);
}

struct RoundDyn {
    int nr;
    int ntA, ntP;
    int pad;
};

struct RoundLists {
    const int *round_ids, *tA0, *tP0;
    struct Tile *tilesA, *tilesP;
    double *hist; size_t lqs;
    unsigned long long *hsize; unsigned int *hcount;
};

struct Tile {
    unsigned long long start;
    unsigned int count;
    unsigned int node;
};

struct QuantBuffers {
    double *buf[2];
    unsigned short *bkt;
    size_t N;
    bool weighted;
};

constexpr int kSum3Slots = 32;
void launch_sum3(const double *planar, size_t N, BinK k, double *d_out6, hipStream_t s);
constexpr int kGqMaxK = 12;
struct GqDpDev {
    unsigned long long w0[kBuckets + 1];
    double w1[3][kBuckets + 1], w2[kBuckets + 1];
    double E[2][kBuckets + 1];
    int cut[kGqMaxK + 1][kBuckets + 1];
};
void launch_gq_dp(const double *d_hist, const unsigned int *d_hcount, int kmax, GqDpDev *d_g, hipStream_t s);

void launch_minmax(const QuantBuffers &qb, const Tile *d_tiles, int ntiles, size_t px, NodeDev *d_nodes, hipStream_t s, bool from_end = false,
                   const RoundDyn *dyn = nullptr, const double *px_src = nullptr, const RoundLists *lists = nullptr);
void launch_hist(const QuantBuffers &qb, bool gq, const Tile *d_tiles, int ntiles, size_t px, NodeDev *d_nodes,
                 double *d_hist, unsigned long long *d_hsize, unsigned int *d_hcount, hipStream_t s, bool from_end = false,
                 bool fixed_point = false, const RoundDyn *dyn = nullptr, const double *px_src = nullptr);
void launch_cut(bool weighted, NodeDev *d_nodes, const int *d_round_nodes, int nround, const double *d_hist,
                const unsigned long long *d_hsize, const unsigned int *d_hcount, unsigned char *d_lut, hipStream_t s,
                const RoundDyn *dyn = nullptr, const double *nr_src = nullptr);
void launch_partition(const QuantBuffers &qb, const Tile *d_ptiles, int nptiles, size_t px, const int *d_round_nodes,
                      const int *d_node_tile0, int nround, NodeDev *d_nodes, const unsigned char *d_lut,
                      unsigned int *d_tilecnt, unsigned long long *d_tileoff, bool fuse_cov, hipStream_t s,
                      bool invariant = false, bool from_end = false, const RoundDyn *dyn = nullptr, const double *px_src = nullptr,
                      bool gated = false);
void launch_cov_children(const QuantBuffers &qb, const Tile *d_tiles, int ntiles, size_t px, NodeDev *d_nodes, hipStream_t s, bool from_end = false,
                         bool gated = false);
void launch_cov_nodes(const QuantBuffers &qb, const double *planar_override, const Tile *d_tiles, int ntiles, size_t px,
                      NodeDev *d_nodes, hipStream_t s, bool from_end = false);

extern std::atomic<int> g_debug_fault;
size_t hist_slot_doubles();

}
```

patolette_amd/csrc/quant.hip:

```cpp
#include "quant.h"

#include <atomic>

#include <type_traits>

namespace pamd {

template <typename T>
__device__ __forceinline__ T block_scan_incl(T v, T *smem) {
    const int lane = threadIdx.x & 63, wid = threadIdx.x >> 6, nw = blockDim.x >> 6;
#pragma unroll
    for (int o = 1; o < 64; o <<= 1) {
        T t = __shfl_up(v, o, 64);
        if (lane >= o) v += t;
    }
    __syncthreads();
    if (lane == 63) smem[wid] = v;
    __syncthreads();
    if (wid == 0) {
        T s = lane < nw ? smem[lane] : T(0);
#pragma unroll
        for (int o = 1; o < 16; o <<= 1) {
            T t = __shfl_up(s, o, 64);
            if (lane >= o) s += t;
        }
        if (lane < nw) smem[lane] = s;
    }
    __syncthreads();
    if (wid > 0) v += smem[wid - 1];
    return v;
}
template <typename T, int N>
__device__ __forceinline__ void block_scan_incl_vec(T (&v)[N], T *smem) {
    const int lane = threadIdx.x & 63, wid = threadIdx.x >> 6, nw = blockDim.x >> 6;
#pragma unroll
    for (int o = 1; o < 64; o <<= 1) {
#pragma unroll
        for (int i = 0; i < N; i++) { T t = __shfl_up(v[i], o, 64); if (lane >= o) v[i] += t; }
    }
    __syncthreads();
    if (lane == 63) {
#pragma unroll
        for (int i = 0; i < N; i++) smem[i * 16 + wid] = v[i];
    }
    __syncthreads();
    if (wid == 0 && lane < 16 * N) {
        const int i = lane >> 4, e = lane & 15;
        T s = (i < N && e < nw) ? smem[i * 16 + e] : T(0);
#pragma unroll
        for (int o = 1; o < 16; o <<= 1) { T t = __shfl_up(s, o, 16); if (e >= o) s += t; }
        if (i < N && e < nw) smem[i * 16 + e] = s;
    }
    __syncthreads();
    if (wid > 0) {
#pragma unroll
        for (int i = 0; i < N; i++) v[i] += smem[i * 16 + wid - 1];
    }
}

__global__ __launch_bounds__(256) void k_sum3(const double *__restrict__ c, size_t N, BinK k, double *out6) {
    __shared__ double sm[6 * 4];
    double a[6] = {0, 0, 0, 0, 0, 0};
    const size_t stride = (size_t)gridDim.x * blockDim.x;
    for (size_t i = (size_t)blockIdx.x * blockDim.x + threadIdx.x; i < N; i += stride) {
        bin_add(c[i], k, a[0], a[1]);
        bin_add(c[N + i], k, a[2], a[3]);
        bin_add(c[2 * N + i], k, a[4], a[5]);
    }
    block_sum<6>(a, sm);
    if (threadIdx.x == 0)
        for (int q = 0; q < 6; q++) unsafeAtomicAdd(&out6[(blockIdx.x & (kSum3Slots - 1)) * 6 + q], a[q]);
}

__device__ __forceinline__ double project(double x, double y, double z, const double a0, const double a1, const double a2) {
    return (x * a0 + y * a1) + z * a2;
}

__device__ __forceinline__ int tile_node(const int *t0, int nr, int t) {
    int lo = 0, hi = nr;
    while (hi - lo > 1) { const int mid = (lo + hi) >> 1; if (t0[mid] <= t) lo = mid; else hi = mid; }
    return lo;
}
template <bool LISTS>
__global__ __launch_bounds__(256) void k_minmax(QuantBuffers qb, const Tile *__restrict__ tiles, NodeDev *nodes, const int from_end,
                                                const RoundDyn *__restrict__ dyn, const RoundLists L) {
    const unsigned nt = dyn ? (unsigned)dyn->ntA : gridDim.x;
    if (blockIdx.x >= nt) return;
    const unsigned tix = from_end ? nt - 1u - blockIdx.x : blockIdx.x;
    Tile t;
    if constexpr (LISTS) {
        const int nr = dyn->nr, ntP = dyn->ntP;
        {
            const int r = tile_node(L.tA0, nr, (int)tix);
            const int id = L.round_ids[r];
            const unsigned long long o = (unsigned long long)((int)tix - L.tA0[r]) * kTileA, n = nodes[id].n;
            t = Tile{nodes[id].begin + o, (unsigned)(n - o < (unsigned long long)kTileA ? n - o : kTileA), (unsigned)id};
            if (threadIdx.x == 0) L.tilesA[tix] = t;
        }
        for (int tp = (int)blockIdx.x + (int)threadIdx.x * (int)nt; tp < ntP; tp += (int)nt * 256) {
            const int r = tile_node(L.tP0, nr, tp);
            const int id = L.round_ids[r];
            const unsigned long long o = (unsigned long long)(tp - L.tP0[r]) * kTileP, n = nodes[id].n;
            L.tilesP[tp] = Tile{nodes[id].begin + o, (unsigned)(n - o < (unsigned long long)kTileP ? n - o : kTileP), (unsigned)id};
        }
        const size_t nh = L.lqs * (size_t)nr, nb = (size_t)nr * kBuckets;
        for (size_t i = (size_t)blockIdx.x * 256 + threadIdx.x; i < nh; i += (size_t)nt * 256) L.hist[i] = 0.0;
        for (size_t i = (size_t)blockIdx.x * 256 + threadIdx.x; i < nb; i += (size_t)nt * 256) { L.hsize[i] = 0ULL; L.hcount[i] = 0u; }
    } else {
        t = tiles[tix];
    }
    NodeDev &nd = nodes[t.node];
    const double a0 = nd.axis[0], a1 = nd.axis[1], a2 = nd.axis[2];
    const double *px = qb.buf[nd.buf], *py = px + qb.N, *pz = py + qb.N;
    double mn = INFINITY, mx = -INFINITY;
    unsigned i = threadIdx.x;
    for (; i + 3 * 256 < t.count; i += 4 * 256) {
        const size_t p = t.start + i;
        double x[4], y[4], z[4];
#pragma unroll
        for (int u = 0; u < 4; u++) { x[u] = px[p + u * 256]; y[u] = py[p + u * 256]; z[u] = pz[p + u * 256]; }
#pragma unroll
        for (int u = 0; u < 4; u++) {
            double d = project(x[u], y[u], z[u], a0, a1, a2);
            mn = fmin(mn, d); mx = fmax(mx, d);
        }
    }
    for (; i < t.count; i += 256) {
        size_t p = t.start + i;
        double d = project(px[p], py[p], pz[p], a0, a1, a2);
        mn = fmin(mn, d); mx = fmax(mx, d);
    }
#pragma unroll
    for (int o = 32; o > 0; o >>= 1) { mn = fmin(mn, __shfl_down(mn, o, 64)); mx = fmax(mx, __shfl_down(mx, o, 64)); }
    __shared__ double smn[4], smx[4];
    if ((threadIdx.x & 63) == 0) { smn[threadIdx.x >> 6] = mn; smx[threadIdx.x >> 6] = mx; }
    __syncthreads();
    if (threadIdx.x == 0) {
        for (int w = 1; w < 4; w++) { mn = fmin(mn, smn[w]); mx = fmax(mx, smx[w]); }
        if (mn <= mx) {
            atomicMin(&nd.minkey[blockIdx.x & (kSlots - 1)], f64_key(mn));
            atomicMax(&nd.maxkey[blockIdx.x & (kSlots - 1)], f64_key(mx));
        }
    }
}

constexpr int kHistCombineMin = 12;
template <bool W, bool GQ>
__global__ __launch_bounds__(512) void k_hist(QuantBuffers qb, const Tile *__restrict__ tiles, int ntiles, NodeDev *nodes,
                                              double *hist, unsigned long long *hsize, unsigned int *hcount, const int from_end,
                                              const RoundDyn *__restrict__ dyn) {
    constexpr int NQ = GQ ? (W ? 14 : 10) : (W ? 4 : 3);
    int nblk = (int)gridDim.x;
    if (dyn) {
        ntiles = dyn->ntA;
        nblk = min(ntiles, nblk);
        if ((int)blockIdx.x >= nblk) return;
    }
    constexpr int NQS = GQ ? kNQ_GQ : kNQ_LQ;
    extern __shared__ double lds[];
    double *h = lds;
    unsigned long long *siz = (unsigned long long *)(h + NQ * 2 * kBuckets);
    unsigned int *cnt = (unsigned int *)(siz + kBuckets);
    for (int i = threadIdx.x; i < NQ * 2 * kBuckets; i += blockDim.x) h[i] = 0.0;
    for (int i = threadIdx.x; i < kBuckets; i += blockDim.x) { cnt[i] = 0u; siz[i] = 0ULL; }
    __syncthreads();

    const int per = (ntiles + nblk - 1) / nblk;
    const int bid = from_end ? nblk - 1 - (int)blockIdx.x : (int)blockIdx.x;
    const int tfirst = bid * per, tlast = min(ntiles, tfirst + per);
    for (int ti = tfirst; ti < tlast; ti++) {
        const Tile t = tiles[ti];
        NodeDev &nd = nodes[t.node];
        const double a0 = nd.axis[0], a1 = nd.axis[1], a2 = nd.axis[2];
        double mn, mx;
        node_minmax(nd, mn, mx);
        const bool degenerate = (mx - mn < kDelta);
        const double sc = 1 / (mx - mn);
        const BinK klin = nd.klin, kquad = nd.kquad;
        const double *px = qb.buf[nd.buf], *py = px + qb.N, *pz = py + qb.N, *pw = pz + qb.N;
        const unsigned long long gslot0 = nd.gslot0;
        if (threadIdx.x == 0) nd.degenerate = degenerate ? 1 : 0;

        auto one = [&](const size_t p, const double x, const double y, const double z, const double w) {
            unsigned b;
            if (degenerate) {
                b = (unsigned)((p - nd.begin + gslot0) % kBuckets);
            } else {
                double ratio = (project(x, y, z, a0, a1, a2) - mn) * sc;
                unsigned long long bq = (unsigned long long)((double)kBuckets * ratio);
                b = bq < (unsigned long long)(kBuckets - 1) ? (unsigned)bq : (unsigned)(kBuckets - 1);
            }
            qb.bkt[p] = (unsigned short)b;
            double pv[2 * NQ];
#define HPART(q, val, K) bin_split((val), (K), pv[2 * (q)], pv[2 * (q) + 1])
            if constexpr (!GQ) {
                HPART(0, x * w, klin); HPART(1, y * w, klin); HPART(2, z * w, klin);
                if constexpr (W) HPART(3, w, klin);
            } else {
                HPART(0, x, klin); HPART(1, y, klin); HPART(2, z, klin);
                HPART(3, (x * x + y * y) + z * z, kquad);
                HPART(4, x * x, kquad); HPART(5, x * y, kquad); HPART(6, y * y, kquad);
                HPART(7, x * z, kquad); HPART(8, y * z, kquad); HPART(9, z * z, kquad);
                if constexpr (W) { HPART(10, x * w, klin); HPART(11, y * w, klin); HPART(12, z * w, klin); HPART(13, w, klin); }
            }
#undef HPART
            unsigned long long wi = 0ULL;
            if constexpr (W && !GQ) wi = (unsigned long long)w;
            bool direct = true;
            if (__ballot(true) == ~0ULL) {
                unsigned long long left = ~0ULL;
#pragma unroll 1
                for (int g = 0; g < 3 && left != 0ULL; g++) {
                    const int first = __builtin_ctzll(left);
                    const unsigned b0 = (unsigned)__builtin_amdgcn_readlane((int)b, first);
                    const bool mine = direct && b == b0;
                    const unsigned long long m = __ballot(mine);
                    if (__popcll(m) < kHistCombineMin) break;
#pragma unroll
                    for (int k2 = 0; k2 < 2 * NQ; k2++) {
                        const double sum = wave_sum_dpp63(mine ? pv[k2] : 0.0);
                        if ((threadIdx.x & 63) == 63) unsafeAtomicAdd(&h[k2 * kBuckets + b0], sum);
                    }
                    if constexpr (W && !GQ) {
                        unsigned long long sw2 = mine ? wi : 0ULL;
#pragma unroll
                        for (int o = 32; o > 0; o >>= 1) sw2 += __shfl_down(sw2, o, 64);
                        if ((threadIdx.x & 63) == 0) atomicAdd(&siz[b0], sw2);
                    }
                    if ((threadIdx.x & 63) == 0) atomicAdd(&cnt[b0], (unsigned)__popcll(m));
                    if (mine) direct = false;
                    left &= ~m;
                }
            }
            if (direct) {
                atomicAdd(&cnt[b], 1u);
#pragma unroll
                for (int k2 = 0; k2 < 2 * NQ; k2++) unsafeAtomicAdd(&h[k2 * kBuckets + b], pv[k2]);
                if constexpr (W && !GQ) atomicAdd(&siz[b], wi);
            }
        };
        unsigned i = threadIdx.x;
        for (; i + 512 < t.count; i += 1024) {
            const size_t p0 = t.start + i, p1 = p0 + 512;
            const double x0 = px[p0], y0 = py[p0], z0 = pz[p0], x1 = px[p1], y1 = py[p1], z1 = pz[p1];
            double w0 = 1.0, w1 = 1.0;
            if constexpr (W) { w0 = pw[p0]; w1 = pw[p1]; }
            one(p0, x0, y0, z0, w0);
            one(p1, x1, y1, z1, w1);
        }
        for (; i < t.count; i += 512) {
            const size_t p = t.start + i;
            double w = 1.0;
            if constexpr (W) w = pw[p];
            one(p, px[p], py[p], pz[p], w);
        }
        const bool flush = (ti + 1 == tlast) || tiles[ti + 1].node != t.node;
        if (!flush) continue;
        __syncthreads();
        const size_t slot = (size_t)nd.slot;
        double *gh = hist + slot * (size_t)(NQS * 2 * kBuckets);
        for (int i = threadIdx.x; i < NQ * 2 * kBuckets; i += blockDim.x) {
            double v = h[i];
            if (v != 0.0) { unsafeAtomicAdd(&gh[i], v); h[i] = 0.0; }
        }
        for (int b = threadIdx.x; b < kBuckets; b += blockDim.x) {
            unsigned c = cnt[b];
            if (c) { atomicAdd(&hcount[slot * kBuckets + b], c); cnt[b] = 0u; }
            if constexpr (W && !GQ) { const unsigned long long s = siz[b]; if (s) { atomicAdd(&hsize[slot * kBuckets + b], s); siz[b] = 0ULL; } }
        }
        __syncthreads();
    }
}

struct FixK { double magic; int s; double ghi, glo; };
__device__ __forceinline__ FixK make_fixk(const BinK k) {
    const int e0 = (int)((__double_as_longlong(k.M0) >> 52) & 0x7ff) - 1023 - 52;
    const int e1 = (int)((__double_as_longlong(k.M1) >> 52) & 0x7ff) - 1023 - 52;
    const int B = e0 - e1, E = e0 + B;
    const int F = 2 * B < 45 ? 2 * B : 45;
    FixK f;
    f.magic = ldexp(1.5, 52 + E - F); f.s = F - B; f.ghi = ldexp(1.0, e0); f.glo = ldexp(1.0, E - F);
    return f;
}
__device__ __forceinline__ long long fix_quant(const double v, const double magic) {
    return __double_as_longlong(v + magic) - __double_as_longlong(magic);
}
template <bool W, bool GQ>
__global__ __launch_bounds__(512) void k_hist_fix(QuantBuffers qb, const Tile *__restrict__ tiles, int ntiles, NodeDev *nodes,
                                              double *hist, unsigned long long *hsize, unsigned int *hcount, const int from_end) {
    constexpr int NQ = GQ ? (W ? 14 : 10) : (W ? 4 : 3);
    constexpr int NQS = GQ ? kNQ_GQ : kNQ_LQ;
    extern __shared__ unsigned long long lds64[];
    unsigned long long *h = lds64;
    unsigned long long *siz = h + NQ * kBuckets;
    unsigned int *cnt = (unsigned int *)(siz + kBuckets);
    for (int i = threadIdx.x; i < NQ * kBuckets; i += blockDim.x) h[i] = 0ULL;
    for (int i = threadIdx.x; i < kBuckets; i += blockDim.x) { cnt[i] = 0u; siz[i] = 0ULL; }
    __syncthreads();

    const int per = (ntiles + (int)gridDim.x - 1) / (int)gridDim.x;
    const int bid = from_end ? (int)gridDim.x - 1 - (int)blockIdx.x : (int)blockIdx.x;
    const int tfirst = bid * per, tlast = min(ntiles, tfirst + per);
    int since_flush = 0;
    for (int ti = tfirst; ti < tlast; ti++) {
        const Tile t = tiles[ti];
        NodeDev &nd = nodes[t.node];
        const double a0 = nd.axis[0], a1 = nd.axis[1], a2 = nd.axis[2];
        double mn, mx;
        node_minmax(nd, mn, mx);
        const bool degenerate = (mx - mn < kDelta);
        const double sc = 1 / (mx - mn);
        const FixK flin = make_fixk(nd.klin), fquad = make_fixk(nd.kquad);
        const double *px = qb.buf[nd.buf], *py = px + qb.N, *pz = py + qb.N, *pw = pz + qb.N;
        const unsigned long long gslot0 = nd.gslot0;
        if (threadIdx.x == 0) nd.degenerate = degenerate ? 1 : 0;

        auto one = [&](const size_t p, const double x, const double y, const double z, const double w) {
            unsigned b;
            if (degenerate) {
                b = (unsigned)((p - nd.begin + gslot0) % kBuckets);
            } else {
                double ratio = (project(x, y, z, a0, a1, a2) - mn) * sc;
                unsigned long long bq = (unsigned long long)((double)kBuckets * ratio);
                b = bq < (unsigned long long)(kBuckets - 1) ? (unsigned)bq : (unsigned)(kBuckets - 1);
            }
            qb.bkt[p] = (unsigned short)b;
            double pv[NQ], pm[NQ];
#define HPART(q, val, K) pv[q] = (val); pm[q] = (K).magic
            if constexpr (!GQ) {
                HPART(0, x * w, flin); HPART(1, y * w, flin); HPART(2, z * w, flin);
                if constexpr (W) { HPART(3, w, flin); }
            } else {
                HPART(0, x, flin); HPART(1, y, flin); HPART(2, z, flin);
                HPART(3, (x * x + y * y) + z * z, fquad);
                HPART(4, x * x, fquad); HPART(5, x * y, fquad); HPART(6, y * y, fquad);
                HPART(7, x * z, fquad); HPART(8, y * z, fquad); HPART(9, z * z, fquad);
                if constexpr (W) { HPART(10, x * w, flin); HPART(11, y * w, flin); HPART(12, z * w, flin); HPART(13, w, flin); }
            }
#undef HPART
            unsigned long long wi = 0ULL;
            if constexpr (W && !GQ) wi = (unsigned long long)w;
            bool direct = true;
            if (__ballot(true) == ~0ULL) {
                unsigned long long left = ~0ULL;
#pragma unroll 1
                for (int g = 0; g < 3 && left != 0ULL; g++) {
                    const int first = __builtin_ctzll(left);
                    const unsigned b0 = (unsigned)__builtin_amdgcn_readlane((int)b, first);
                    const bool mine = direct && b == b0;
                    const unsigned long long m = __ballot(mine);
                    if (__popcll(m) < kHistCombineMin) break;
#pragma unroll
                    for (int k2 = 0; k2 < NQ; k2++) {
                        const double vq = (pv[k2] + pm[k2]) - pm[k2];
                        const double sum = wave_sum_dpp63(mine ? vq : 0.0);
                        if ((threadIdx.x & 63) == 63) atomicAdd(&h[k2 * kBuckets + b0], (unsigned long long)fix_quant(sum, pm[k2]));
                    }
                    if constexpr (W && !GQ) {
                        unsigned long long sw2 = mine ? wi : 0ULL;
#pragma unroll
                        for (int o = 32; o > 0; o >>= 1) sw2 += __shfl_down(sw2, o, 64);
                        if ((threadIdx.x & 63) == 0) atomicAdd(&siz[b0], sw2);
                    }
                    if ((threadIdx.x & 63) == 0) atomicAdd(&cnt[b0], (unsigned)__popcll(m));
                    if (mine) direct = false;
                    left &= ~m;
                }
            }
            if (direct) {
                atomicAdd(&cnt[b], 1u);
#pragma unroll
                for (int k2 = 0; k2 < NQ; k2++) atomicAdd(&h[k2 * kBuckets + b], (unsigned long long)fix_quant(pv[k2], pm[k2]));
                if constexpr (W && !GQ) atomicAdd(&siz[b], wi);
            }
        };
        unsigned i = threadIdx.x;
        for (; i + 512 < t.count; i += 1024) {
            const size_t p0 = t.start + i, p1 = p0 + 512;
            const double x0 = px[p0], y0 = py[p0], z0 = pz[p0], x1 = px[p1], y1 = py[p1], z1 = pz[p1];
            double w0 = 1.0, w1 = 1.0;
            if constexpr (W) { w0 = pw[p0]; w1 = pw[p1]; }
            one(p0, x0, y0, z0, w0);
            one(p1, x1, y1, z1, w1);
        }
        for (; i < t.count; i += 512) {
            const size_t p = t.start + i;
            double w = 1.0;
            if constexpr (W) w = pw[p];
            one(p, px[p], py[p], pz[p], w);
        }
        since_flush++;
        const bool flush = (ti + 1 == tlast) || tiles[ti + 1].node != t.node || since_flush >= 16;
        if (!flush) continue;
        since_flush = 0;
        __syncthreads();
        const size_t slot = (size_t)nd.slot;
        double *gh = hist + slot * (size_t)(NQS * 2 * kBuckets);
        for (int i2 = threadIdx.x; i2 < NQ * kBuckets; i2 += blockDim.x) {
            const long long S = (long long)h[i2];
            if (S != 0) {
                const int q = i2 / kBuckets, bb = i2 % kBuckets;
                const bool quad = GQ && q >= 3 && q <= 9;
                const FixK &f = quad ? fquad : flin;
                const long long Sh = (S + (1LL << (f.s - 1))) >> f.s, Sl = S - (Sh << f.s);
                if (Sh != 0) unsafeAtomicAdd(&gh[(q * 2 + 0) * kBuckets + bb], (double)Sh * f.ghi);
                if (Sl != 0) unsafeAtomicAdd(&gh[(q * 2 + 1) * kBuckets + bb], (double)Sl * f.glo);
                h[i2] = 0ULL;
            }
        }
        for (int b = threadIdx.x; b < kBuckets; b += blockDim.x) {
            unsigned c = cnt[b];
            if (c) { atomicAdd(&hcount[slot * kBuckets + b], c); cnt[b] = 0u; }
            if constexpr (W && !GQ) { const unsigned long long s2 = siz[b]; if (s2) { atomicAdd(&hsize[slot * kBuckets + b], s2); siz[b] = 0ULL; } }
        }
        __syncthreads();
    }
}

template <bool W>
__global__ __launch_bounds__(512) void k_cut(NodeDev *nodes, const int *__restrict__ round_nodes, const double *__restrict__ hist,
                                             const unsigned long long *__restrict__ hsize, const unsigned int *__restrict__ hcount,
                                             unsigned char *lut, const int fault, const RoundDyn *__restrict__ dyn) {
    if (dyn && (int)blockIdx.x >= dyn->nr) return;
    __shared__ double sd[4 * 16];
    __shared__ unsigned long long su[2 * 16];
    __shared__ double best_v[8];
    __shared__ int best_i[8];
    __shared__ double tot[8];
    __shared__ unsigned long long tots[2];
    __shared__ int s_split;
    const int b = threadIdx.x;
    NodeDev &nd = nodes[round_nodes[blockIdx.x]];
    const size_t slot = (size_t)nd.slot;
    const double *gh = hist + slot * (size_t)(kNQ_LQ * 2 * kBuckets);
    constexpr int NQ = W ? 4 : 3;
    double p[NQ][2];
    {
        double v0[NQ], v1[NQ];
#pragma unroll
        for (int q = 0; q < NQ; q++) { v0[q] = gh[(q * 2 + 0) * kBuckets + b]; v1[q] = gh[(q * 2 + 1) * kBuckets + b]; }
        block_scan_incl_vec<double, NQ>(v0, sd);
        block_scan_incl_vec<double, NQ>(v1, sd);
#pragma unroll
        for (int q = 0; q < NQ; q++) { p[q][0] = v0[q]; p[q][1] = v1[q]; }
    }
    unsigned long long cs[2] = {(unsigned long long)hcount[slot * kBuckets + b], W ? hsize[slot * kBuckets + b] : 0ULL};
    block_scan_incl_vec<unsigned long long, 2>(cs, su);
    const unsigned long long cnt = cs[0], siz = W ? cs[1] : cs[0];
    __syncthreads();
    if (b == kBuckets - 1) {
#pragma unroll
        for (int q = 0; q < NQ; q++) { tot[q * 2] = p[q][0]; tot[q * 2 + 1] = p[q][1]; }
        tots[0] = cnt; tots[1] = siz;
    }
    __syncthreads();
    double obj = 0;
    {
        const double sl = (double)siz, sr = (double)tots[1] - sl;
#pragma unroll
        for (int j = 0; j < 3; j++) {
            double csl = p[j][0] + p[j][1];
            double csr = (tot[j * 2] + tot[j * 2 + 1]) - csl;
            double v = 0;
            if (sl != 0) v += (csl * csl) / sl;
            if (sr != 0) v += (csr * csr) / sr;
            obj += v;
        }
    }
    double bv = obj; int bi = b;
#pragma unroll
    for (int o = 32; o > 0; o >>= 1) {
        double ov = __shfl_down(bv, o, 64); int oi = __shfl_down(bi, o, 64);
        if (ov > bv || (ov == bv && (fault == 3 ? oi > bi : oi < bi))) { bv = ov; bi = oi; }
    }
    if ((b & 63) == 0) { best_v[b >> 6] = bv; best_i[b >> 6] = bi; }
    __syncthreads();
    if (b == 0) {
        for (int w = 1; w < 8; w++)
            if (best_v[w] > bv || (best_v[w] == bv && (fault == 3 ? best_i[w] > bi : best_i[w] < bi))) { bv = best_v[w]; bi = best_i[w]; }
        if (fault == 1) {
            unsigned long long upto = 0;
            for (int i = 0; i <= bi; i++) upto += hcount[slot * kBuckets + i];
            int b2 = bi + 1;
            while (b2 < kBuckets - 1 && hcount[slot * kBuckets + b2] == 0u) b2++;
            if (b2 < kBuckets - 1 && upto + hcount[slot * kBuckets + b2] < tots[0]) bi = b2;
        }
        s_split = bi;
    }
    __syncthreads();
    const int split = s_split;
    lut[slot * kBuckets + b] = b > split ? 1 : 0;
    if (b == split) {
        nd.split = split;
        const unsigned long long nL = cnt, nR = tots[0] - cnt;
        nd.cbegin[0] = nd.begin; nd.cbegin[1] = nd.begin + nL; nd.cbegin[2] = nd.begin + nd.n;
        for (int side = 0; side < 2; side++) {
            NodeDev &ch = nodes[nd.child0 + side];
            ch.begin = side == 0 ? nd.begin : nd.begin + nL;
            ch.n = side == 0 ? nL : nR;
            ch.gn = ch.n;
            ch.buf = 1 - nd.buf;
            ch.slot = -1; ch.child0 = -1; ch.nchild = 0;
            ch.klin = nd.klin; ch.kquad = nd.kquad;
            ch.psplit = split | (nd.degenerate ? 0x10000 : 0);
            double s0[NQ], s1[NQ];
#pragma unroll
            for (int q = 0; q < NQ; q++) {
                s0[q] = side == 0 ? p[q][0] : tot[q * 2] - p[q][0];
                s1[q] = side == 0 ? p[q][1] : tot[q * 2 + 1] - p[q][1];
            }
            double sw = W ? (s0[NQ - 1] + s1[NQ - 1]) : (double)ch.n;
            ch.sw = sw;
            const double inv = 1 / sw;
            for (int j = 0; j < 3; j++) ch.mean[j] = (s0[j] + s1[j]) * inv;
            ch.axis[0] = ch.axis[1] = ch.axis[2] = 0;
        }
    }
    for (int i = b; i < 2 * kNodeResetElems; i += kBuckets)
        node_reset_element(nodes[nd.child0 + i / kNodeResetElems], i % kNodeResetElems);
}

__global__ __launch_bounds__(256) void k_count(QuantBuffers qb, const Tile *__restrict__ tiles, const NodeDev *__restrict__ nodes,
                                               const unsigned char *__restrict__ lut, unsigned int *tilecnt, const int from_end,
                                               const RoundDyn *__restrict__ dyn) {
    __shared__ unsigned int c[kMaxChildren];
    __shared__ unsigned char sl[kBuckets];
    const unsigned nt = dyn ? (unsigned)dyn->ntP : gridDim.x;
    if (blockIdx.x >= nt) return;
    const unsigned tix = from_end ? nt - 1u - blockIdx.x : blockIdx.x;
    const Tile t = tiles[tix];
    const NodeDev &nd = nodes[t.node];
    const unsigned char *l = lut + (size_t)nd.slot * kBuckets;
    if (threadIdx.x < kMaxChildren) c[threadIdx.x] = 0;
    const int nch = nd.nchild;
    typedef unsigned short us8 __attribute__((ext_vector_type(8), aligned(2)));
    const int split = nd.split;
    if (nch == 2 && split >= 0) {
        const unsigned i0 = threadIdx.x * 8u;
        unsigned right = 0;
        if (i0 + 8u <= t.count) {
            const us8 v = *reinterpret_cast<const us8 *>(qb.bkt + t.start + i0);
#pragma unroll
            for (int j = 0; j < 8; j++) right += (int)v[j] > split ? 1u : 0u;
        } else {
            for (unsigned i = i0; i < t.count && i < i0 + 8u; i++) right += (int)qb.bkt[t.start + i] > split ? 1u : 0u;
        }
        __syncthreads();
        right = wave_sum_u32(right);
        if ((threadIdx.x & 63) == 0 && right) atomicAdd(&c[1], right);
        __syncthreads();
        if (threadIdx.x == 0) c[0] = t.count - c[1];
        __syncthreads();
    } else if (nch == 2) {
        for (int b = threadIdx.x; b < kBuckets; b += blockDim.x) sl[b] = l[b];
        __syncthreads();
        const unsigned i0 = threadIdx.x * 8u;
        unsigned right = 0;
        if (i0 + 8u <= t.count) {
            const us8 v = *reinterpret_cast<const us8 *>(qb.bkt + t.start + i0);
#pragma unroll
            for (int j = 0; j < 8; j++) right += sl[v[j]];
        } else {
            for (unsigned i = i0; i < t.count && i < i0 + 8u; i++) right += sl[qb.bkt[t.start + i]];
        }
        right = wave_sum_u32(right);
        if ((threadIdx.x & 63) == 0 && right) atomicAdd(&c[1], right);
        __syncthreads();
        if (threadIdx.x == 0) c[0] = t.count - c[1];
        __syncthreads();
    } else {
        __syncthreads();
        for (unsigned i = threadIdx.x; i < ((t.count + 255u) & ~255u); i += blockDim.x) {
            int child = i < t.count ? (int)l[qb.bkt[t.start + i]] : 255;
            for (int k = 0; k < nch; k++) {
                unsigned long long m = __ballot(child == k);
                if ((threadIdx.x & 63) == 0 && m) atomicAdd(&c[k], (unsigned)__popcll(m));
            }
        }
        __syncthreads();
    }
    if (threadIdx.x < kMaxChildren) tilecnt[(size_t)tix * kMaxChildren + threadIdx.x] = c[threadIdx.x];
}
__global__ __launch_bounds__(1024) void k_scan(const int *__restrict__ round_nodes, const int *__restrict__ node_tile0, NodeDev *nodes,
                                              const unsigned int *__restrict__ tilecnt, unsigned long long *tileoff,
                                              const RoundDyn *__restrict__ dyn) {
    if (dyn && (int)blockIdx.x >= dyn->nr) return;
    __shared__ unsigned long long su[16];
    __shared__ unsigned long long total;
    NodeDev &nd = nodes[round_nodes[blockIdx.x]];
    const int t0 = node_tile0[blockIdx.x], t1 = node_tile0[blockIdx.x + 1];
    const int C = (t1 - t0 + (int)blockDim.x - 1) / (int)blockDim.x;
    const int a = t0 + (int)threadIdx.x * C, b = min(t1, a + C);
    unsigned long long base = nd.begin;
    const int nch = nd.nchild;
    if (nch == 2) {
        __shared__ unsigned long long sv[2 * 16];
        __shared__ unsigned long long tot2[2];
        unsigned long long sum[2] = {0, 0};
        for (int g = a; g < b; g += 8) {
            uint2 v[8];
#pragma unroll
            for (int q = 0; q < 8; q++) v[q] = g + q < b ? *reinterpret_cast<const uint2 *>(tilecnt + (size_t)(g + q) * kMaxChildren) : make_uint2(0u, 0u);
#pragma unroll
            for (int q = 0; q < 8; q++) { sum[0] += v[q].x; sum[1] += v[q].y; }
        }
        unsigned long long inc[2] = {sum[0], sum[1]};
        block_scan_incl_vec<unsigned long long, 2>(inc, sv);
        if (threadIdx.x == blockDim.x - 1) { tot2[0] = inc[0]; tot2[1] = inc[1]; }
        __syncthreads();
        const unsigned long long base1 = base + tot2[0];
        unsigned long long run0 = base + inc[0] - sum[0], run1 = base1 + inc[1] - sum[1];
        for (int g = a; g < b; g += 8) {
            uint2 v[8];
#pragma unroll
            for (int q = 0; q < 8; q++) v[q] = g + q < b ? *reinterpret_cast<const uint2 *>(tilecnt + (size_t)(g + q) * kMaxChildren) : make_uint2(0u, 0u);
#pragma unroll
            for (int q = 0; q < 8; q++) {
                if (g + q < b) *reinterpret_cast<ulonglong2 *>(tileoff + (size_t)(g + q) * kMaxChildren) = make_ulonglong2(run0, run1);
                run0 += v[q].x; run1 += v[q].y;
            }
        }
        if (threadIdx.x == 0) { nd.cbegin[0] = base; nd.cbegin[1] = base1; nd.cbegin[2] = base1 + tot2[1]; }
        return;
    }
    for (int k = 0; k < nch; k++) {
        unsigned long long sum = 0;
        for (int g = a; g < b; g += 8) {
            unsigned v[8];
#pragma unroll
            for (int q = 0; q < 8; q++) v[q] = g + q < b ? tilecnt[(size_t)(g + q) * kMaxChildren + k] : 0u;
#pragma unroll
            for (int q = 0; q < 8; q++) sum += v[q];
        }
        const unsigned long long inc = block_scan_incl<unsigned long long>(sum, su);
        if (threadIdx.x == blockDim.x - 1) total = inc;
        unsigned long long run = base + inc - sum;
        for (int g = a; g < b; g += 8) {
            unsigned v[8];
#pragma unroll
            for (int q = 0; q < 8; q++) v[q] = g + q < b ? tilecnt[(size_t)(g + q) * kMaxChildren + k] : 0u;
#pragma unroll
            for (int q = 0; q < 8; q++) {
                if (g + q < b) tileoff[(size_t)(g + q) * kMaxChildren + k] = run;
                run += v[q];
            }
        }
        if (threadIdx.x == 0) nd.cbegin[k] = base;
        __syncthreads();
        base += total;
        __syncthreads();
    }
    if (threadIdx.x == 0) nd.cbegin[nch] = base;
}

template <bool W>
__global__ __launch_bounds__(256, 5) void k_scatter(QuantBuffers qb, const Tile *__restrict__ tiles, int ntiles, NodeDev *nodes,
                                                    const unsigned char *__restrict__ lut, const unsigned long long *__restrict__ tileoff,
                                                    const int from_end) {
    constexpr int R = kTileP / 256;
    __shared__ unsigned long long off[R][4][kMaxChildren];
    const int lane = threadIdx.x & 63, wid = threadIdx.x >> 6;
    const unsigned long long ltmask = (1ULL << lane) - 1ULL;
    if ((from_end & 4) && nodes[0].nchild == 2) return;
    const int per = (ntiles + (int)gridDim.x - 1) / (int)gridDim.x;
    const int bid = (from_end & 1) ? (int)gridDim.x - 1 - (int)blockIdx.x : (int)blockIdx.x;
    const int tfirst = bid * per, tlast = min(ntiles, tfirst + per);
    for (int ti = tfirst; ti < tlast; ti++) {
        const Tile t = tiles[ti];
        const NodeDev &nd = nodes[t.node];
        const unsigned char *l = lut + (size_t)nd.slot * kBuckets;
        const int nch = nd.nchild;
        unsigned cr[R];
#pragma unroll
        for (int r = 0; r < R; r++) {
            unsigned i = r * 256 + threadIdx.x;
            int ch = 255;
            if (i < t.count) ch = (int)l[qb.bkt[t.start + i]];
            unsigned rk = 0;
            for (int k = 0; k < nch; k++) {
                unsigned long long m = __ballot(ch == k);
                if (ch == k) rk = (unsigned)__popcll(m & ltmask);
                if (lane == 0) off[r][wid][k] = (unsigned long long)__popcll(m);
            }
            cr[r] = (unsigned)ch | (rk << 8);
        }
        __syncthreads();
        if ((int)threadIdx.x < nch) {
            unsigned long long run = tileoff[(size_t)ti * kMaxChildren + threadIdx.x];
            for (int r = 0; r < R; r++)
                for (int w = 0; w < 4; w++) { unsigned long long c = off[r][w][threadIdx.x]; off[r][w][threadIdx.x] = run; run += c; }
        }
        __syncthreads();
        const double *sx = qb.buf[nd.buf], *sy = sx + qb.N, *sz = sy + qb.N, *sw = sz + qb.N;
        double *dx = qb.buf[1 - nd.buf], *dy = dx + qb.N, *dz = dy + qb.N, *dw = dz + qb.N;
#pragma unroll
        for (int r = 0; r < R; r++) {
            const int ch = (int)(cr[r] & 255u);
            if (ch != 255) {
                const size_t src = t.start + r * 256 + threadIdx.x;
                const size_t dst = off[r][wid][ch] + (cr[r] >> 8);
                const double x = sx[src], y = sy[src], z = sz[src];
                double w = 1.0;
                if constexpr (W) w = sw[src];
                dx[dst] = x; dy[dst] = y; dz[dst] = z;
                if constexpr (W) dw[dst] = w;
            }
        }
        __syncthreads();
    }
}

template <bool W, bool INV>
__global__ __launch_bounds__(256, (W || INV) ? 2 : 3) void k_scatter_bin(QuantBuffers qb, const Tile *__restrict__ tiles, int ntiles, NodeDev *nodes,
                                                                        const NodeDev *__restrict__ nodes_ro,
                                                                        const unsigned long long *__restrict__ tileoff, const int from_end,
                                                                        const RoundDyn *__restrict__ dyn) {
    constexpr int R = kTileP / 256;
    static_assert(R * 4 == 32, "one 32-lane group per child");
    __shared__ unsigned int wcnt[2][2][R * 4];
    __shared__ double sm[28 * 4];
    const int lane = threadIdx.x & 63, wid = __builtin_amdgcn_readfirstlane((int)(threadIdx.x >> 6));
    const unsigned long long ltmask = (1ULL << lane) - 1ULL;
    int nblk = (int)gridDim.x;
    if ((from_end & 2) && nodes_ro[0].nchild != 2) return;
    if (dyn) {
        ntiles = dyn->ntP;
        nblk = min(ntiles, nblk);
        if ((int)blockIdx.x >= nblk) return;
    }
    const int per = (ntiles + nblk - 1) / nblk;
    const int bid = (from_end & 1) ? nblk - 1 - (int)blockIdx.x : (int)blockIdx.x;
    const int tfirst = bid * per, tlast = min(ntiles, tfirst + per);
    if (tfirst >= tlast) return;
    constexpr int NP = INV ? 14 : 7;
    double pl[NP], pr[NP];
#pragma unroll
    for (int i = 0; i < NP; i++) { pl[i] = 0; pr[i] = 0; }

    auto fetch_buckets = [&](const Tile &tt, const int ti, unsigned (&b)[R], unsigned long long &toff) {
        const unsigned last = tt.count - 1u;
#pragma unroll
        for (int r = 0; r < R; r++) b[r] = qb.bkt[tt.start + min((unsigned)(r * 256) + threadIdx.x, last)];
        toff = tileoff[(size_t)ti * kMaxChildren + (lane >> 5)];
    };
    auto classify = [&](const Tile &tt, const unsigned (&b)[R], const int split, const int par, unsigned (&cr)[R]) {
#pragma unroll
        for (int r = 0; r < R; r++) {
            const bool valid = (unsigned)(r * 256) + threadIdx.x < tt.count;
            const bool right = (int)b[r] > split;
            const unsigned long long mR = __ballot(valid && right), mL = __ballot(valid && !right);
            const unsigned rk = (unsigned)__popcll((right ? mR : mL) & ltmask);
            cr[r] = (valid ? (right ? 1u : 0u) : 2u) | (rk << 8);
            if (lane == 0) { wcnt[par][0][r * 4 + wid] = (unsigned)__popcll(mL); wcnt[par][1][r * 4 + wid] = (unsigned)__popcll(mR); }
        }
    };
    auto lane64 = [](const unsigned long long v, const int l) {
        return ((unsigned long long)(unsigned)__builtin_amdgcn_readlane((int)(unsigned)(v >> 32), l) << 32) |
               (unsigned)__builtin_amdgcn_readlane((int)(unsigned)v, l);
    };
    Tile t = tiles[tfirst];
    unsigned cr[R];
    unsigned long long baseL, baseR;
    {
        unsigned b0[R];
        unsigned long long toff;
        fetch_buckets(t, tfirst, b0, toff);
        classify(t, b0, nodes_ro[t.node].split, 0, cr);
        baseL = lane64(toff, 0); baseR = lane64(toff, 32);
    }
    for (int ti = tfirst; ti < tlast; ti++) {
        const int par = (ti - tfirst) & 1;
        const NodeDev &nd = nodes_ro[t.node];
        const int child0 = nd.child0;
        const double *sx = qb.buf[nd.buf], *sy = sx + qb.N, *sz = sy + qb.N, *sw = sz + qb.N;
        double *dx = qb.buf[1 - nd.buf], *dy = dx + qb.N, *dz = dy + qb.N, *dw = dz + qb.N;
        double x[R], y[R], z[R], w[R];
        {
            const unsigned last = t.count - 1u;
#pragma unroll
            for (int r = 0; r < R; r++) {
                const size_t src = t.start + min((unsigned)(r * 256) + threadIdx.x, last);
                x[r] = sx[src]; y[r] = sy[src]; z[r] = sz[src];
                w[r] = 1.0;
                if constexpr (W) w[r] = sw[src];
            }
        }
        const bool more = ti + 1 < tlast;
        const int tnx = more ? ti + 1 : ti;
        const Tile tn = tiles[tnx];
        unsigned bkn[R];
        unsigned long long toffn;
        fetch_buckets(tn, tnx, bkn, toffn);
        __syncthreads();
        const unsigned c = wcnt[par][lane >> 5][lane & 31];
        const unsigned incl = wave_scan_incl_u32(c);
        const unsigned tot0 = (unsigned)__builtin_amdgcn_readlane((int)incl, 31);
        const unsigned excl = incl - c - (lane >= 32 ? tot0 : 0u);
        const NodeDev &c0 = nodes_ro[child0], &c1 = nodes_ro[child0 + 1];
        const double m0L = c0.mean[0], m1L = c0.mean[1], m2L = c0.mean[2], m0R = c1.mean[0], m1R = c1.mean[1], m2R = c1.mean[2];
        BinK kinv{0.0, 0.0};
        if constexpr (INV) kinv = nd.kquad;
        const size_t slack = (size_t)(W ? 4 : 3) * qb.N + (size_t)lane;
#pragma unroll
        for (int r = 0; r < R; r++) {
            const unsigned eL = (unsigned)__builtin_amdgcn_readlane((int)excl, r * 4 + wid);
            const unsigned eR = (unsigned)__builtin_amdgcn_readlane((int)excl, 32 + r * 4 + wid);
            const unsigned ch = cr[r] & 255u;
            const bool right = ch == 1u, none = ch == 2u;
            const size_t dst = (right ? baseR + eR : baseL + eL) + (cr[r] >> 8);
            dx[none ? slack : dst] = x[r]; dy[none ? slack - qb.N : dst] = y[r]; dz[none ? slack - 2 * qb.N : dst] = z[r];
            if constexpr (W) dw[none ? slack - 3 * qb.N : dst] = w[r];
            const double rf = right ? 1.0 : 0.0, lf = ch == 0u ? 1.0 : 0.0;
            const double ex = x[r] - (right ? m0R : m0L), ey = y[r] - (right ? m1R : m1L), ez = z[r] - (right ? m2R : m2L);
            const double wx = w[r] * ex, wy = w[r] * ey, wz = w[r] * ez;
            const double q[7] = {wx * ex, wy * ex, wz * ex, wy * ey, wz * ey, wz * ez, ((ex * ex + ey * ey) + ez * ez) * w[r]};
            if constexpr (INV) {
#pragma unroll
                for (int i = 0; i < 7; i++) {
                    double v0, v1;
                    bin_split(q[i], kinv, v0, v1);
                    pl[2 * i] = __builtin_fma(v0, lf, pl[2 * i]); pl[2 * i + 1] = __builtin_fma(v1, lf, pl[2 * i + 1]);
                    pr[2 * i] = __builtin_fma(v0, rf, pr[2 * i]); pr[2 * i + 1] = __builtin_fma(v1, rf, pr[2 * i + 1]);
                }
            } else {
#pragma unroll
                for (int i = 0; i < 7; i++) { pl[i] = __builtin_fma(q[i], lf, pl[i]); pr[i] = __builtin_fma(q[i], rf, pr[i]); }
            }
        }
        const bool flush = !more || tn.node != t.node;
        if (flush) {
            const BinK kq = nd.kquad;
            double a[28];
            if constexpr (INV) {
#pragma unroll
                for (int i = 0; i < 14; i++) { a[i] = pl[i]; a[14 + i] = pr[i]; pl[i] = 0; pr[i] = 0; }
            } else {
#pragma unroll
                for (int i = 0; i < 7; i++) {
                    bin_split(pl[i], kq, a[2 * i], a[2 * i + 1]);
                    bin_split(pr[i], kq, a[14 + 2 * i], a[14 + 2 * i + 1]);
                    pl[i] = 0; pr[i] = 0;
                }
            }
            block_sum<28>(a, sm);
            if (threadIdx.x == 0) {
                for (int side = 0; side < 2; side++) {
                    NodeDev &chn = nodes[child0 + side];
                    for (int i = 0; i < 7; i++) {
                        if (a[14 * side + 2 * i] != 0.0) unsafeAtomicAdd(&chn.acc[blockIdx.x & (kSlots - 1)][i][0], a[14 * side + 2 * i]);
                        if (a[14 * side + 2 * i + 1] != 0.0) unsafeAtomicAdd(&chn.acc[blockIdx.x & (kSlots - 1)][i][1], a[14 * side + 2 * i + 1]);
                    }
                }
            }
        }
        if (more) {
            classify(tn, bkn, nodes_ro[tn.node].split, par ^ 1, cr);
            baseL = lane64(toffn, 0); baseR = lane64(toffn, 32);
        }
        t = tn;
    }
}

template <bool W>
__device__ __forceinline__ void cov_accumulate(const double *px, const double *py, const double *pz, const double *pw,
                                               size_t lo, size_t hi, const double m0, const double m1, const double m2,
                                               const BinK kq, double (&a)[14]) {
    for (size_t p = lo + threadIdx.x; p < hi; p += blockDim.x) {
        double dx = px[p] - m0, dy = py[p] - m1, dz = pz[p] - m2;
        double w = 1.0;
        if constexpr (W) w = pw[p];
        double wx = w * dx, wy = w * dy, wz = w * dz;
        bin_add(wx * dx, kq, a[0], a[1]);
        bin_add(wy * dx, kq, a[2], a[3]);
        bin_add(wz * dx, kq, a[4], a[5]);
        bin_add(wy * dy, kq, a[6], a[7]);
        bin_add(wz * dy, kq, a[8], a[9]);
        bin_add(wz * dz, kq, a[10], a[11]);
        bin_add(((dx * dx + dy * dy) + dz * dz) * w, kq, a[12], a[13]);
    }
}

template <bool W>
__global__ __launch_bounds__(256) void k_cov_children(QuantBuffers qb, const Tile *__restrict__ tiles, NodeDev *nodes, const int from_end) {
    __shared__ double sm[14 * 4];
    if ((from_end & 4) && nodes[0].nchild == 2) return;
    const Tile t = tiles[(from_end & 1) ? gridDim.x - 1u - blockIdx.x : blockIdx.x];
    const NodeDev &nd = nodes[t.node];
    const double *px = qb.buf[1 - nd.buf], *py = px + qb.N, *pz = py + qb.N, *pw = pz + qb.N;
    const size_t t_lo = t.start, t_hi = t.start + t.count;
    for (int k = 0; k < nd.nchild; k++) {
        size_t lo = nd.cbegin[k] > t_lo ? nd.cbegin[k] : t_lo;
        size_t hi = nd.cbegin[k + 1] < t_hi ? nd.cbegin[k + 1] : t_hi;
        if (lo >= hi) continue;
        NodeDev &ch = nodes[nd.child0 + k];
        double a[14];
#pragma unroll
        for (int i = 0; i < 14; i++) a[i] = 0;
        cov_accumulate<W>(px, py, pz, pw, lo, hi, ch.mean[0], ch.mean[1], ch.mean[2], nd.kquad, a);
        block_sum<14>(a, sm);
        if (threadIdx.x == 0)
            for (int q = 0; q < 7; q++) { unsafeAtomicAdd(&ch.acc[blockIdx.x & (kSlots - 1)][q][0], a[2 * q]); unsafeAtomicAdd(&ch.acc[blockIdx.x & (kSlots - 1)][q][1], a[2 * q + 1]); }
    }
}

template <bool W>
__global__ __launch_bounds__(256) void k_cov_nodes(QuantBuffers qb, const double *planar, const Tile *__restrict__ tiles, NodeDev *nodes,
                                                   const int from_end) {
    __shared__ double sm[14 * 4];
    const Tile t = tiles[from_end ? gridDim.x - 1u - blockIdx.x : blockIdx.x];
    NodeDev &nd = nodes[t.node];
    const double *px = planar ? planar : qb.buf[nd.buf], *py = px + qb.N, *pz = py + qb.N, *pw = pz + qb.N;
    double a[14];
#pragma unroll
    for (int i = 0; i < 14; i++) a[i] = 0;
    cov_accumulate<W>(px, py, pz, pw, t.start, t.start + t.count, nd.mean[0], nd.mean[1], nd.mean[2], nd.kquad, a);
    block_sum<14>(a, sm);
    if (threadIdx.x == 0)
        for (int q = 0; q < 7; q++) { unsafeAtomicAdd(&nd.acc[blockIdx.x & (kSlots - 1)][q][0], a[2 * q]); unsafeAtomicAdd(&nd.acc[blockIdx.x & (kSlots - 1)][q][1], a[2 * q + 1]); }
}

size_t hist_slot_doubles() { return (size_t)kNQ_GQ * 2 * kBuckets; }

void launch_sum3(const double *planar, size_t N, BinK k, double *d_out6, hipStream_t s) {
    HIP_CHECK(hipMemsetAsync(d_out6, 0, kSum3Slots * 6 * sizeof(double), s));
    size_t g = ceil_div(N, 256 * 16);
    if (g > 2048) g = 2048;
    if (g < 1) g = 1;
    KTIME("k_sum3", s, 24.0 * N);
    hipLaunchKernelGGL(k_sum3, (int)g, 256, 0, s, planar, N, k, d_out6);
    HIP_CHECK(hipGetLastError());
}

void launch_minmax(const QuantBuffers &qb, const Tile *d_tiles, int ntiles, size_t px, NodeDev *d_nodes, hipStream_t s, bool from_end,
                   const RoundDyn *dyn, const double *px_src, const RoundLists *lists) {
    if (!ntiles) return;
    KTIME_DYN("k_minmax", s, 24.0, px, px_src);
    if (dyn && lists) hipLaunchKernelGGL(k_minmax<true>, ntiles, 256, 0, s, qb, d_tiles, d_nodes, from_end ? 1 : 0, dyn, *lists);
    else hipLaunchKernelGGL(k_minmax<false>, ntiles, 256, 0, s, qb, d_tiles, d_nodes, from_end ? 1 : 0, dyn, RoundLists{});
    HIP_CHECK(hipGetLastError());
}

template <bool W>
static void launch_hist_fix(const QuantBuffers &qb, const Tile *d_tiles, int ntiles, size_t px, NodeDev *d_nodes, double *d_hist,
                            unsigned long long *d_hsize, unsigned int *d_hcount, hipStream_t s, bool from_end) {
    constexpr int NQ = W ? 14 : 10;
    const size_t lds = (size_t)NQ * kBuckets * sizeof(unsigned long long) + kBuckets * (sizeof(unsigned int) + sizeof(unsigned long long));
    static PerDeviceOnce attr_set;
    if (attr_set.first()) HIP_CHECK(hipFuncSetAttribute((const void *)k_hist_fix<W, true>, hipFuncAttributeMaxDynamicSharedMemorySize, (int)lds));
    KTIME("k_hist_gq", s, (W ? 34.0 : 26.0) * px);
    const int g = std::min(ntiles, 256 * (W ? 2 : 3));
    hipLaunchKernelGGL((k_hist_fix<W, true>), g, 512, lds, s, qb, d_tiles, ntiles, d_nodes, d_hist, d_hsize, d_hcount, from_end ? 1 : 0);
    HIP_CHECK(hipGetLastError());
}

template <bool W, bool GQ>
static void launch_hist_t(const QuantBuffers &qb, const Tile *d_tiles, int ntiles, size_t px, NodeDev *d_nodes, double *d_hist,
                          unsigned long long *d_hsize, unsigned int *d_hcount, hipStream_t s, bool from_end,
                          const RoundDyn *dyn = nullptr, const double *px_src = nullptr) {
    constexpr int NQ = GQ ? (W ? 14 : 10) : (W ? 4 : 3);
    size_t lds = (size_t)NQ * 2 * kBuckets * sizeof(double) + kBuckets * (sizeof(unsigned int) + sizeof(unsigned long long));
    static PerDeviceOnce attr_set;
    if (attr_set.first()) HIP_CHECK(hipFuncSetAttribute((const void *)k_hist<W, GQ>, hipFuncAttributeMaxDynamicSharedMemorySize, (int)lds));
    KTIME_DYN(GQ ? "k_hist_gq" : "k_hist_lq", s, (W ? 34.0 : 26.0), px, px_src);
    const int g = std::min(ntiles, 256 * (GQ ? 1 : 4));
    hipLaunchKernelGGL((k_hist<W, GQ>), g, 512, lds, s, qb, d_tiles, ntiles, d_nodes, d_hist, d_hsize, d_hcount, from_end ? 1 : 0, dyn);
    HIP_CHECK(hipGetLastError());
}

__global__ __launch_bounds__(512) void k_gq_prefix(const double *__restrict__ hist, const unsigned int *__restrict__ hcount, GqDpDev *g) {
    __shared__ double sh[4][kBuckets + 1];
    __shared__ unsigned long long sc[kBuckets + 1];
    const int b = threadIdx.x;
#pragma unroll
    for (int hq = 0; hq < 4; hq++)
        sh[hq][b + 1] = hist[(size_t)(hq * 2 + 0) * kBuckets + b] + hist[(size_t)(hq * 2 + 1) * kBuckets + b];
    sc[b + 1] = hcount[b];
    if (b < 4) sh[b][0] = 0;
    if (b == 4) sc[0] = 0;
    __syncthreads();
    if (b == 0) { unsigned long long a = 0; for (int i = 1; i <= kBuckets; i++) { a += sc[i]; sc[i] = a; } }
    else if ((b & 63) == 0 && b <= 256) {
        double *t = sh[(b >> 6) - 1];
        double a = 0;
        for (int i = 1; i <= kBuckets; i++) { a = t[i] + a; t[i] = a; }
    }
    __syncthreads();
    for (int i = b; i <= kBuckets; i += 512) {
        g->w0[i] = sc[i];
        g->w1[0][i] = sh[0][i]; g->w1[1][i] = sh[1][i]; g->w1[2][i] = sh[2][i]; g->w2[i] = sh[3][i];
    }
}
__device__ __forceinline__ double gq_distortion(const GqDpDev *g, int a, int b) {
    if (g->w0[a] == g->w0[b]) return 0;
    const double q0 = g->w1[0][b] - g->w1[0][a], q1 = g->w1[1][b] - g->w1[1][a], q2 = g->w1[2][b] - g->w1[2][a];
    return g->w2[b] - g->w2[a] - (q0 * q0 + q1 * q1 + q2 * q2) / (double)(g->w0[b] - g->w0[a]);
}
__global__ void k_gq_init(GqDpDev *g) {
    const int i = blockIdx.x * blockDim.x + threadIdx.x;
    if (i <= kBuckets) g->E[0][i] = i >= 1 ? gq_distortion(g, 0, i) : 0.0;
}
__global__ __launch_bounds__(256) void k_gq_dp(GqDpDev *g, int k) {
    const int n = (int)blockIdx.x;
    const double *Ep = g->E[k & 1];
    double *En = g->E[(k & 1) ^ 1];
    if (n < k + 1) { if (threadIdx.x == 0) En[n] = Ep[n]; return; }
    double best = INFINITY; int bt = -1;
    for (int t = n - 2 - (int)threadIdx.x; t >= k - 1; t -= (int)blockDim.x) {
        const double v = Ep[t] + gq_distortion(g, t, n);
        if (v < best) { best = v; bt = t; }
    }
    __shared__ double sv[256];
    __shared__ int st[256];
    sv[threadIdx.x] = best; st[threadIdx.x] = bt;
    __syncthreads();
    for (int o = 128; o > 0; o >>= 1) {
        if ((int)threadIdx.x < o) {
            const double v2 = sv[threadIdx.x + o]; const int t2 = st[threadIdx.x + o];
            const double v1 = sv[threadIdx.x]; const int t1 = st[threadIdx.x];
            if (t2 >= 0 && (t1 < 0 || v2 < v1 || (v2 == v1 && t2 > t1))) { sv[threadIdx.x] = v2; st[threadIdx.x] = t2; }
        }
        __syncthreads();
    }
    if (threadIdx.x == 0) {
        double e = Ep[n - 1]; int cut = n - 1;
        if (st[0] >= 0 && sv[0] < e) { e = sv[0]; cut = st[0]; }
        En[n] = e;
        g->cut[k][n] = cut;
    }
}

void launch_gq_dp(const double *d_hist, const unsigned int *d_hcount, int kmax, GqDpDev *d_g, hipStream_t s) {
    KTIME("k_gq_dp", s, (double)kmax * 513 * 513 * 8);
    hipLaunchKernelGGL(k_gq_prefix, 1, 512, 0, s, d_hist, d_hcount, d_g);
    hipLaunchKernelGGL(k_gq_init, 3, 256, 0, s, d_g);
    for (int k = 2; k <= kmax; k++) hipLaunchKernelGGL(k_gq_dp, kBuckets + 1, 256, 0, s, d_g, k);
    HIP_CHECK(hipGetLastError());
}

void launch_hist(const QuantBuffers &qb, bool gq, const Tile *d_tiles, int ntiles, size_t px, NodeDev *d_nodes,
                 double *d_hist, unsigned long long *d_hsize, unsigned int *d_hcount, hipStream_t s, bool from_end, bool fixed_point,
                 const RoundDyn *dyn, const double *px_src) {
    if (!ntiles) return;
    if (gq && fixed_point) {
        if (qb.weighted) launch_hist_fix<true>(qb, d_tiles, ntiles, px, d_nodes, d_hist, d_hsize, d_hcount, s, from_end);
        else launch_hist_fix<false>(qb, d_tiles, ntiles, px, d_nodes, d_hist, d_hsize, d_hcount, s, from_end);
        return;
    }
    if (qb.weighted) { if (gq) launch_hist_t<true, true>(qb, d_tiles, ntiles, px, d_nodes, d_hist, d_hsize, d_hcount, s, from_end);
                       else launch_hist_t<true, false>(qb, d_tiles, ntiles, px, d_nodes, d_hist, d_hsize, d_hcount, s, from_end, dyn, px_src); }
    else { if (gq) launch_hist_t<false, true>(qb, d_tiles, ntiles, px, d_nodes, d_hist, d_hsize, d_hcount, s, from_end);
           else launch_hist_t<false, false>(qb, d_tiles, ntiles, px, d_nodes, d_hist, d_hsize, d_hcount, s, from_end, dyn, px_src); }
}

std::atomic<int> g_debug_fault{0};
void launch_cut(bool weighted, NodeDev *d_nodes, const int *d_round_nodes, int nround, const double *d_hist,
                const unsigned long long *d_hsize, const unsigned int *d_hcount, unsigned char *d_lut, hipStream_t s, const RoundDyn *dyn, const double *nr_src) {
    if (!nround) return;
    KTIME_DYN("k_cut", s, (double)kNQ_LQ * 2 * kBuckets * 8, nround, nr_src);
    const int fault = g_debug_fault.load(std::memory_order_relaxed);
    if (weighted) hipLaunchKernelGGL(k_cut<true>, nround, 512, 0, s, d_nodes, d_round_nodes, d_hist, d_hsize, d_hcount, d_lut, fault, dyn);
    else hipLaunchKernelGGL(k_cut<false>, nround, 512, 0, s, d_nodes, d_round_nodes, d_hist, d_hsize, d_hcount, d_lut, fault, dyn);
    HIP_CHECK(hipGetLastError());
}

void launch_partition(const QuantBuffers &qb, const Tile *d_ptiles, int nptiles, size_t px, const int *d_round_nodes,
                      const int *d_node_tile0, int nround, NodeDev *d_nodes, const unsigned char *d_lut,
                      unsigned int *d_tilecnt, unsigned long long *d_tileoff, bool fuse_cov, hipStream_t s, bool invariant, bool from_end,
                      const RoundDyn *dyn, const double *px_src, bool gated) {
    const int fe = (from_end ? 1 : 0) | (gated ? 2 : 0);
    if (!nround) return;
    if (nptiles) { KTIME_DYN("k_count", s, 2.0, px, px_src); hipLaunchKernelGGL(k_count, nptiles, 256, 0, s, qb, d_ptiles, d_nodes, d_lut, d_tilecnt, fe & 1, dyn); }
    { KTIME_DYN("k_scan", s, 12.0 * kMaxChildren / (double)kTileP, dyn ? px : (size_t)nptiles * kTileP, px_src);
      hipLaunchKernelGGL(k_scan, nround, 1024, 0, s, d_round_nodes, d_node_tile0, d_nodes, d_tilecnt, d_tileoff, dyn); }
    if (nptiles) {
        KTIME_DYN(fuse_cov ? "k_scatter_cov" : "k_scatter", s, (qb.weighted ? 66.0 : 50.0), px, px_src);
        if (fuse_cov) {
            const int gb = std::min(nptiles, 256 * ((invariant || qb.weighted) ? 2 : 3));
            if (invariant) {
                if (qb.weighted) hipLaunchKernelGGL((k_scatter_bin<true, true>), gb, 256, 0, s, qb, d_ptiles, nptiles, d_nodes, (const NodeDev *)d_nodes, d_tileoff, fe, dyn);
                else hipLaunchKernelGGL((k_scatter_bin<false, true>), gb, 256, 0, s, qb, d_ptiles, nptiles, d_nodes, (const NodeDev *)d_nodes, d_tileoff, fe, dyn);
            } else if (qb.weighted) hipLaunchKernelGGL((k_scatter_bin<true, false>), gb, 256, 0, s, qb, d_ptiles, nptiles, d_nodes, (const NodeDev *)d_nodes, d_tileoff, fe, dyn);
            else hipLaunchKernelGGL((k_scatter_bin<false, false>), gb, 256, 0, s, qb, d_ptiles, nptiles, d_nodes, (const NodeDev *)d_nodes, d_tileoff, fe, dyn);
            if (gated) {
                HIP_CHECK(hipGetLastError());
                const int fg = (from_end ? 1 : 0) | 4;
                if (qb.weighted) hipLaunchKernelGGL((k_scatter<true>), nptiles, 256, 0, s, qb, d_ptiles, nptiles, d_nodes, d_lut, d_tileoff, fg);
                else hipLaunchKernelGGL((k_scatter<false>), nptiles, 256, 0, s, qb, d_ptiles, nptiles, d_nodes, d_lut, d_tileoff, fg);
            }
        } else {
            if (qb.weighted) hipLaunchKernelGGL((k_scatter<true>), nptiles, 256, 0, s, qb, d_ptiles, nptiles, d_nodes, d_lut, d_tileoff, fe);
            else hipLaunchKernelGGL((k_scatter<false>), nptiles, 256, 0, s, qb, d_ptiles, nptiles, d_nodes, d_lut, d_tileoff, fe);
        }
    }
    HIP_CHECK(hipGetLastError());
}

void launch_cov_children(const QuantBuffers &qb, const Tile *d_tiles, int ntiles, size_t px, NodeDev *d_nodes, hipStream_t s, bool from_end, bool gated) {
    if (!ntiles) return;
    KTIME("k_cov", s, (qb.weighted ? 32.0 : 24.0) * px);
    const int fe = (from_end ? 1 : 0) | (gated ? 4 : 0);
    if (qb.weighted) hipLaunchKernelGGL(k_cov_children<true>, ntiles, 256, 0, s, qb, d_tiles, d_nodes, fe);
    else hipLaunchKernelGGL(k_cov_children<false>, ntiles, 256, 0, s, qb, d_tiles, d_nodes, fe);
    HIP_CHECK(hipGetLastError());
}

void launch_cov_nodes(const QuantBuffers &qb, const double *planar_override, const Tile *d_tiles, int ntiles, size_t px,
                      NodeDev *d_nodes, hipStream_t s, bool from_end) {
    if (!ntiles) return;
    KTIME("k_cov", s, ((qb.weighted && !planar_override) ? 32.0 : 24.0) * px);
    if (qb.weighted && !planar_override) hipLaunchKernelGGL(k_cov_nodes<true>, ntiles, 256, 0, s, qb, planar_override, d_tiles, d_nodes, from_end ? 1 : 0);
    else hipLaunchKernelGGL(k_cov_nodes<false>, ntiles, 256, 0, s, qb, planar_override, d_tiles, d_nodes, from_end ? 1 : 0);
    HIP_CHECK(hipGetLastError());
}

}
```

Measured before the change: 3211.

## Fold cut and child-moment kernels into hist and scatter via last-block tickets

Removes the separate k_cut launch and the per-round k_lq_children launch. Each hist block now bumps a per-node ticket counter after its atomics, and whichever block finishes the node's last tile runs the cut for that node. The scatter kernel does the same to compute the child moments. This cuts two kernel launches and their serialization from every split round, at the cost of agent-scope atomics, memory drains and extra tail work on the last block of each node.

```diff
diff --git a/patolette_amd/csrc/devutil.h b/patolette_amd/csrc/devutil.h
--- a/patolette_amd/csrc/devutil.h
+++ b/patolette_amd/csrc/devutil.h
@@ -90,6 +90,29 @@
     __syncthreads();
 }
 
+struct LdPlain {
+    template <typename T> static __device__ __forceinline__ T ld(const T *p) { return *p; }
+};
+struct LdAgent {
+    static __device__ __forceinline__ unsigned int ld(const unsigned int *p) { return __hip_atomic_load(p, __ATOMIC_RELAXED, __HIP_MEMORY_SCOPE_AGENT); }
+    static __device__ __forceinline__ unsigned long long ld(const unsigned long long *p) { return __hip_atomic_load(p, __ATOMIC_RELAXED, __HIP_MEMORY_SCOPE_AGENT); }
+    static __device__ __forceinline__ double ld(const double *p) {
+        return __longlong_as_double((long long)__hip_atomic_load(reinterpret_cast<const unsigned long long *>(p), __ATOMIC_RELAXED, __HIP_MEMORY_SCOPE_AGENT));
+    }
+};
+
+__device__ __forceinline__ void wave_drain() { asm volatile("s_waitcnt vmcnt(0)" ::: "memory"); }
+__device__ __forceinline__ bool node_ticket(unsigned int *ticket, const unsigned int share, const unsigned int total) {
+    asm volatile("s_waitcnt vmcnt(0)" ::: "memory");
+    const unsigned int before = __hip_atomic_fetch_add(ticket, share, __ATOMIC_RELAXED, __HIP_MEMORY_SCOPE_AGENT);
+    const bool last = before + share == total;
+    if (last) {
+        __builtin_amdgcn_fence(__ATOMIC_ACQUIRE, "agent");
+        asm volatile("s_waitcnt vmcnt(0)" ::: "memory");
+    }
+    return last;
+}
+
 __host__ __device__ inline unsigned long long f64_key(double d) {
     union { double f; unsigned long long u; } c;
     c.f = d;
diff --git a/patolette_amd/csrc/pipeline.hip b/patolette_amd/csrc/pipeline.hip
--- a/patolette_amd/csrc/pipeline.hip
+++ b/patolette_amd/csrc/pipeline.hip
@@ -178,37 +178,6 @@
 
 struct GqOut { int kbase, error, pad[2]; int cuts[16]; unsigned long long ticks[8]; };
 
-constexpr int kLqDevMaxK = 256;
-constexpr int kLqNodeCap = 16 * kLqDevMaxK + 256;
-constexpr int kLqRoundCap = 512;
-constexpr int kLqMaxRounds = 96;
-
-struct LqRec {
-    double val;
-    int left;
-    int kn;
-};
-struct LqCen { double mean[3]; double gn; };
-struct LqHead {
-    int done, error, rounds, nnodes, neval, pad;
-    unsigned long long split_evals, split_px;
-    double tau;
-    double round_px[kLqMaxRounds], round_nr[kLqMaxRounds];
-};
-struct LqCtl {
-    LqHead h;
-    int K, M, nleaves, pad;
-    int ncids[2];
-    RoundDyn dyn;
-    int leaves[kLqNodeCap];
-    int round_ids[kLqRoundCap];
-    int cids[2][2 * kLqRoundCap];
-    int tA0[kLqRoundCap + 1], tP0[kLqRoundCap + 1];
-    int nparent[kLqNodeCap];
-    double np[kLqNodeCap];
-    LqRec nrec[kLqNodeCap];
-    LqCen ncen[kLqNodeCap];
-};
 template <> struct WsPoison<LqCtl> {
     static void dev(LqCtl *p, size_t a, size_t b) {
         for (size_t i = a; i < b; i++) {
@@ -249,38 +218,7 @@
     if (wave >= ncids) return;
     const int id = init ? init_first + wave : c->cids[call & 1][wave];
     if (init && lane == 0) c->cids[0][wave] = id;
-    NodeDev &d = nodes[id];
-    const double *acc = &d.acc[0][0][0];
-    double sum = 0;
-    if (lane < 14) {
-        double v[kSlots];
-#pragma unroll
-        for (int k = 0; k < kSlots; k++) v[k] = acc[k * 14 + lane];
-#pragma unroll
-        for (int k = 0; k < kSlots; k++) sum += v[k];
-    }
-    const double pair = sum + __shfl_down(sum, 1, 64);
-    double cov[7];
-#pragma unroll
-    for (int q = 0; q < 7; q++)
-        cov[q] = __hiloint2double(__builtin_amdgcn_readlane(__double2hiint(pair), 2 * q), __builtin_amdgcn_readlane(__double2loint(pair), 2 * q));
-    if (lane != 0) return;
-    double ub = cov[6];
-    const bool single = d.gn <= 1ULL;
-    const double sw = d.sw;
-    if (single || !(sw > 0)) ub = 0;
-    else {
-        double c6[6];
-        for (int q = 0; q < 6; q++) c6[q] = cov[q] / sw;
-        const double b = hm::lambda_max_bound(c6) * sw * (1.0 + 1e-9) + 1e-9 * cov[6];
-        if (b == b && b < ub) ub = b;
-    }
-    for (int q = 0; q < 6; q++) d.cov6[q] = cov[q];
-    d.dist = cov[6]; d.ub = ub; d.axis_state = 0;
-    c->nrec[id] = LqRec{single ? 0.0 : ub, -1, single ? 1 : 0};
-    c->nparent[id] = init ? -1 : c->round_ids[wave >> 1];
-    c->ncen[id] = LqCen{{d.mean[0], d.mean[1], d.mean[2]}, (double)d.gn};
-    c->leaves[(init ? 0 : c->nleaves) + wave] = id;
+    lq_child_moments<LdPlain>(nodes, c, id, wave, init);
 }
 
 __device__ __forceinline__ int block_excl_scan_256(const int v, int *sw , int &total) {
@@ -492,7 +430,7 @@
     out[t] = tr;
 }
 
-__global__ __launch_bounds__(256) void k_round_setup_dyn(NodeDev *table, const LqCtl *c, Tile *tilesA, Tile *tilesP, double *hist,
+__global__ __launch_bounds__(256) void k_round_setup_dyn(NodeDev *table, LqCtl *c, Tile *tilesA, Tile *tilesP, double *hist,
                                                          unsigned long long *hsize, unsigned int *hcount, const size_t lqs) {
     const int nr = c->dyn.nr;
     if (nr == 0) return;
@@ -514,6 +452,7 @@
     }
     for (size_t i = tid; i < lqs * (size_t)nr; i += stride) hist[i] = 0.0;
     for (size_t i = tid; i < (size_t)nr * kBuckets; i += stride) { hsize[i] = 0ULL; hcount[i] = 0u; }
+    for (size_t i = tid; i < (size_t)nr; i += stride) { c->ticket[0][i] = 0u; c->ticket[1][i] = 0u; }
 }
 
 struct GqTab {
@@ -1321,33 +1260,33 @@
     const int kb_ub = kbase < 0 ? kGqMaxK : kbase;
     auto control = [&]() {
         const bool first = call == 0;
-        {
+        if (first) {
             KTIME("k_lq_children", s, 0.0);
-            if (first) hipLaunchKernelGGL(k_lq_children, (kb_ub + 3) / 4, 256, 0, s, E.nodes.p, c, call, kb_ub, first_base, nnodes, (int)K, gq);
-            else hipLaunchKernelGGL(k_lq_children, 2 * kLqRoundCap / 4, 256, 0, s, E.nodes.p, c, call, 0, 0, 0, 0, (const GqOut *)nullptr);
+            hipLaunchKernelGGL(k_lq_children, (kb_ub + 3) / 4, 256, 0, s, E.nodes.p, c, call, kb_ub, first_base, nnodes, (int)K, gq);
         }
         KTIME("k_lq_select", s, 0.0);
         hipLaunchKernelGGL(k_lq_select, 1 + (first ? (kb_ub + 3) / 4 : 2 * kLqRoundCap / 4), 256, 0, s, E.nodes.p, c, call, bnd.e_lin, bnd.e_quad);
         HIP_CHECK(hipGetLastError());
         call++;
     };
+    const RoundFold fold{c, E.lut.p};
     int enq = 0;
     auto round = [&]() {
         if (enq >= kLqMaxRounds) throw HipError("patolette_amd: split loop exceeded its round limit");
-        const double *px_src = &head->round_px[enq], *nr_src = &head->round_nr[enq];
+        const double *px_src = &head->round_px[enq];
         const bool rev = enq % 2 == 1;
         static const bool setup_kernel = getenv("PAMD_LQ_SETUP_KERNEL") && atoi(getenv("PAMD_LQ_SETUP_KERNEL")) != 0;
         if (setup_kernel) {
-            hipLaunchKernelGGL(k_round_setup_dyn, 1024, 256, 0, s, E.nodes.p, (const LqCtl *)c, E.tilesA.p, E.tilesP.p, E.hist.p, E.hsize.p, E.hcount.p, lqs);
+            hipLaunchKernelGGL(k_round_setup_dyn, 1024, 256, 0, s, E.nodes.p, c, E.tilesA.p, E.tilesP.p, E.hist.p, E.hsize.p, E.hcount.p, lqs);
             HIP_CHECK(hipGetLastError());
             launch_minmax(qlq, E.tilesA.p, ntA_ub, 0, E.nodes.p, s, rev, dyn, px_src);
         } else {
-            const RoundLists rl{c->round_ids, c->tA0, c->tP0, E.tilesA.p, E.tilesP.p, E.hist.p, lqs, E.hsize.p, E.hcount.p};
+            const RoundLists rl{c->round_ids, c->tA0, c->tP0, E.tilesA.p, E.tilesP.p, E.hist.p, lqs, E.hsize.p, E.hcount.p, &c->ticket[0][0]};
             launch_minmax(qlq, E.tilesA.p, ntA_ub, 0, E.nodes.p, s, rev, dyn, px_src, &rl);
         }
-        launch_hist(qlq, false, E.tilesA.p, ntA_ub, 0, E.nodes.p, E.hist.p, E.hsize.p, E.hcount.p, s, !rev, false, dyn, px_src);
-        launch_cut(weighted, E.nodes.p, d_round, kLqRoundCap, E.hist.p, E.hsize.p, E.hcount.p, E.lut.p, s, dyn, nr_src);
-        launch_partition(qlq, E.tilesP.p, ntP_ub, 0, d_round, d_tP0, kLqRoundCap, E.nodes.p, E.lut.p, E.tilecnt.p, E.tileoff.p, true, s, inv_sums, rev, dyn, px_src);
+        launch_hist(qlq, false, E.tilesA.p, ntA_ub, 0, E.nodes.p, E.hist.p, E.hsize.p, E.hcount.p, s, !rev, false, dyn, px_src, &fold);
+        launch_partition(qlq, E.tilesP.p, ntP_ub, 0, d_round, d_tP0, kLqRoundCap, E.nodes.p, E.lut.p, E.tilecnt.p, E.tileoff.p, true, s, inv_sums, rev, dyn, px_src,
+                         false, &fold);
         enq++;
         control();
     };
diff --git a/patolette_amd/csrc/quant.h b/patolette_amd/csrc/quant.h
--- a/patolette_amd/csrc/quant.h
+++ b/patolette_amd/csrc/quant.h
@@ -4,6 +4,7 @@
 
 #include "common.h"
 #include "devutil.h"
+#include "host_math.h"
 
 namespace pamd {
 
@@ -92,7 +93,81 @@
     struct Tile *tilesA, *tilesP;
     double *hist; size_t lqs;
     unsigned long long *hsize; unsigned int *hcount;
-};
+    unsigned int *ticket;
+};
+struct RoundFold {
+    struct LqCtl *ctl;
+    unsigned char *lut;
+};
+
+constexpr int kLqDevMaxK = 256;
+constexpr int kLqNodeCap = 16 * kLqDevMaxK + 256;
+constexpr int kLqRoundCap = 512;
+constexpr int kLqMaxRounds = 96;
+
+struct LqRec {
+    double val;
+    int left;
+    int kn;
+};
+struct LqCen { double mean[3]; double gn; };
+struct LqHead {
+    int done, error, rounds, nnodes, neval, pad;
+    unsigned long long split_evals, split_px;
+    double tau;
+    double round_px[kLqMaxRounds], round_nr[kLqMaxRounds];
+};
+struct LqCtl {
+    LqHead h;
+    int K, M, nleaves, pad;
+    int ncids[2];
+    RoundDyn dyn;
+    unsigned int ticket[2][kLqRoundCap];
+    int leaves[kLqNodeCap];
+    int round_ids[kLqRoundCap];
+    int cids[2][2 * kLqRoundCap];
+    int tA0[kLqRoundCap + 1], tP0[kLqRoundCap + 1];
+    int nparent[kLqNodeCap];
+    double np[kLqNodeCap];
+    LqRec nrec[kLqNodeCap];
+    LqCen ncen[kLqNodeCap];
+};
+template <class LD>
+__device__ __forceinline__ void lq_child_moments(NodeDev *nodes, LqCtl *c, const int id, const int wave, const bool init) {
+    const int lane = threadIdx.x & 63;
+    NodeDev &d = nodes[id];
+    const double *acc = &d.acc[0][0][0];
+    double sum = 0;
+    if (lane < 14) {
+        double v[kSlots];
+#pragma unroll
+        for (int k = 0; k < kSlots; k++) v[k] = LD::ld(acc + k * 14 + lane);
+#pragma unroll
+        for (int k = 0; k < kSlots; k++) sum += v[k];
+    }
+    const double pair = sum + __shfl_down(sum, 1, 64);
+    double cov[7];
+#pragma unroll
+    for (int q = 0; q < 7; q++)
+        cov[q] = __hiloint2double(__builtin_amdgcn_readlane(__double2hiint(pair), 2 * q), __builtin_amdgcn_readlane(__double2loint(pair), 2 * q));
+    if (lane != 0) return;
+    double ub = cov[6];
+    const bool single = d.gn <= 1ULL;
+    const double sw = d.sw;
+    if (single || !(sw > 0)) ub = 0;
+    else {
+        double c6[6];
+        for (int q = 0; q < 6; q++) c6[q] = cov[q] / sw;
+        const double b = hm::lambda_max_bound(c6) * sw * (1.0 + 1e-9) + 1e-9 * cov[6];
+        if (b == b && b < ub) ub = b;
+    }
+    for (int q = 0; q < 6; q++) d.cov6[q] = cov[q];
+    d.dist = cov[6]; d.ub = ub; d.axis_state = 0;
+    c->nrec[id] = LqRec{single ? 0.0 : ub, -1, single ? 1 : 0};
+    c->nparent[id] = init ? -1 : c->round_ids[wave >> 1];
+    c->ncen[id] = LqCen{{d.mean[0], d.mean[1], d.mean[2]}, (double)d.gn};
+    c->leaves[(init ? 0 : c->nleaves) + wave] = id;
+}
 
 struct Tile {
     unsigned long long start;
@@ -122,7 +197,7 @@
                    const RoundDyn *dyn = nullptr, const double *px_src = nullptr, const RoundLists *lists = nullptr);
 void launch_hist(const QuantBuffers &qb, bool gq, const Tile *d_tiles, int ntiles, size_t px, NodeDev *d_nodes,
                  double *d_hist, unsigned long long *d_hsize, unsigned int *d_hcount, hipStream_t s, bool from_end = false,
-                 bool fixed_point = false, const RoundDyn *dyn = nullptr, const double *px_src = nullptr);
+                 bool fixed_point = false, const RoundDyn *dyn = nullptr, const double *px_src = nullptr, const RoundFold *fold = nullptr);
 void launch_cut(bool weighted, NodeDev *d_nodes, const int *d_round_nodes, int nround, const double *d_hist,
                 const unsigned long long *d_hsize, const unsigned int *d_hcount, unsigned char *d_lut, hipStream_t s,
                 const RoundDyn *dyn = nullptr, const double *nr_src = nullptr);
@@ -130,7 +205,7 @@
                       const int *d_node_tile0, int nround, NodeDev *d_nodes, const unsigned char *d_lut,
                       unsigned int *d_tilecnt, unsigned long long *d_tileoff, bool fuse_cov, hipStream_t s,
                       bool invariant = false, bool from_end = false, const RoundDyn *dyn = nullptr, const double *px_src = nullptr,
-                      bool gated = false);
+                      bool gated = false, const RoundFold *fold = nullptr);
 void launch_cov_children(const QuantBuffers &qb, const Tile *d_tiles, int ntiles, size_t px, NodeDev *d_nodes, hipStream_t s, bool from_end = false,
                          bool gated = false);
 void launch_cov_nodes(const QuantBuffers &qb, const double *planar_override, const Tile *d_tiles, int ntiles, size_t px,
diff --git a/patolette_amd/csrc/quant.hip b/patolette_amd/csrc/quant.hip
--- a/patolette_amd/csrc/quant.hip
+++ b/patolette_amd/csrc/quant.hip
@@ -106,6 +106,7 @@
         const size_t nh = L.lqs * (size_t)nr, nb = (size_t)nr * kBuckets;
         for (size_t i = (size_t)blockIdx.x * 256 + threadIdx.x; i < nh; i += (size_t)nt * 256) L.hist[i] = 0.0;
         for (size_t i = (size_t)blockIdx.x * 256 + threadIdx.x; i < nb; i += (size_t)nt * 256) { L.hsize[i] = 0ULL; L.hcount[i] = 0u; }
+        for (int i = (int)blockIdx.x * 256 + (int)threadIdx.x; i < nr; i += (int)nt * 256) { L.ticket[i] = 0u; L.ticket[kLqRoundCap + i] = 0u; }
     } else {
         t = tiles[tix];
     }
@@ -144,11 +145,15 @@
     }
 }
 
+template <bool W, class LD>
+__device__ __forceinline__ void cut_node(NodeDev *nodes, NodeDev &nd, const double *__restrict__ hist, const unsigned long long *__restrict__ hsize,
+                                         const unsigned int *__restrict__ hcount, unsigned char *lut, const int fault, const int degenerate);
 constexpr int kHistCombineMin = 12;
-template <bool W, bool GQ>
+template <bool W, bool GQ, bool FOLD>
 __global__ __launch_bounds__(512) void k_hist(QuantBuffers qb, const Tile *__restrict__ tiles, int ntiles, NodeDev *nodes,
                                               double *hist, unsigned long long *hsize, unsigned int *hcount, const int from_end,
-                                              const RoundDyn *__restrict__ dyn) {
+                                              const RoundDyn *__restrict__ dyn, const RoundFold fold, const int fault) {
+    static_assert(!FOLD || !GQ, "the cut belongs to the local quantiser's rounds");
     constexpr int NQ = GQ ? (W ? 14 : 10) : (W ? 4 : 3);
     int nblk = (int)gridDim.x;
     if (dyn) {
@@ -168,6 +173,7 @@
     const int per = (ntiles + nblk - 1) / nblk;
     const int bid = from_end ? nblk - 1 - (int)blockIdx.x : (int)blockIdx.x;
     const int tfirst = bid * per, tlast = min(ntiles, tfirst + per);
+    unsigned run = 0;
     for (int ti = tfirst; ti < tlast; ti++) {
         const Tile t = tiles[ti];
         NodeDev &nd = nodes[t.node];
@@ -177,6 +183,7 @@
         const bool degenerate = (mx - mn < kDelta);
         const double sc = 1 / (mx - mn);
         const BinK klin = nd.klin, kquad = nd.kquad;
+        run++;
         const double *px = qb.buf[nd.buf], *py = px + qb.N, *pz = py + qb.N, *pw = pz + qb.N;
         const unsigned long long gslot0 = nd.gslot0;
         if (threadIdx.x == 0) nd.degenerate = degenerate ? 1 : 0;
@@ -268,7 +275,18 @@
             if (c) { atomicAdd(&hcount[slot * kBuckets + b], c); cnt[b] = 0u; }
             if constexpr (W && !GQ) { const unsigned long long s = siz[b]; if (s) { atomicAdd(&hsize[slot * kBuckets + b], s); siz[b] = 0ULL; } }
         }
-        __syncthreads();
+        if constexpr (FOLD) wave_drain();
+        __syncthreads();
+        if constexpr (FOLD) {
+            __shared__ int s_last;
+            if (threadIdx.x == 0) {
+                const LqCtl *c = fold.ctl;
+                s_last = node_ticket(&fold.ctl->ticket[0][slot], run, (unsigned)(c->tA0[slot + 1] - c->tA0[slot])) ? 1 : 0;
+            }
+            run = 0;
+            __syncthreads();
+            if (s_last) cut_node<W, LdAgent>(nodes, nd, hist, hsize, hcount, fold.lut, fault, degenerate ? 1 : 0);
+        }
     }
 }
 
@@ -417,11 +435,10 @@
     }
 }
 
-template <bool W>
-__global__ __launch_bounds__(512) void k_cut(NodeDev *nodes, const int *__restrict__ round_nodes, const double *__restrict__ hist,
-                                             const unsigned long long *__restrict__ hsize, const unsigned int *__restrict__ hcount,
-                                             unsigned char *lut, const int fault, const RoundDyn *__restrict__ dyn) {
-    if (dyn && (int)blockIdx.x >= dyn->nr) return;
+template <bool W, class LD>
+__device__ __forceinline__ void cut_node(NodeDev *nodes, NodeDev &nd, const double *__restrict__ hist,
+                                         const unsigned long long *__restrict__ hsize, const unsigned int *__restrict__ hcount,
+                                         unsigned char *lut, const int fault, const int degenerate) {
     __shared__ double sd[4 * 16];
     __shared__ unsigned long long su[2 * 16];
     __shared__ double best_v[8];
@@ -430,7 +447,6 @@
     __shared__ unsigned long long tots[2];
     __shared__ int s_split;
     const int b = threadIdx.x;
-    NodeDev &nd = nodes[round_nodes[blockIdx.x]];
     const size_t slot = (size_t)nd.slot;
     const double *gh = hist + slot * (size_t)(kNQ_LQ * 2 * kBuckets);
     constexpr int NQ = W ? 4 : 3;
@@ -438,13 +454,13 @@
     {
         double v0[NQ], v1[NQ];
 #pragma unroll
-        for (int q = 0; q < NQ; q++) { v0[q] = gh[(q * 2 + 0) * kBuckets + b]; v1[q] = gh[(q * 2 + 1) * kBuckets + b]; }
+        for (int q = 0; q < NQ; q++) { v0[q] = LD::ld(gh + (q * 2 + 0) * kBuckets + b); v1[q] = LD::ld(gh + (q * 2 + 1) * kBuckets + b); }
         block_scan_incl_vec<double, NQ>(v0, sd);
         block_scan_incl_vec<double, NQ>(v1, sd);
 #pragma unroll
         for (int q = 0; q < NQ; q++) { p[q][0] = v0[q]; p[q][1] = v1[q]; }
     }
-    unsigned long long cs[2] = {(unsigned long long)hcount[slot * kBuckets + b], W ? hsize[slot * kBuckets + b] : 0ULL};
+    unsigned long long cs[2] = {(unsigned long long)LD::ld(hcount + slot * kBuckets + b), W ? LD::ld(hsize + slot * kBuckets + b) : 0ULL};
     block_scan_incl_vec<unsigned long long, 2>(cs, su);
     const unsigned long long cnt = cs[0], siz = W ? cs[1] : cs[0];
     __syncthreads();
@@ -480,10 +496,10 @@
             if (best_v[w] > bv || (best_v[w] == bv && (fault == 3 ? best_i[w] > bi : best_i[w] < bi))) { bv = best_v[w]; bi = best_i[w]; }
         if (fault == 1) {
             unsigned long long upto = 0;
-            for (int i = 0; i <= bi; i++) upto += hcount[slot * kBuckets + i];
+            for (int i = 0; i <= bi; i++) upto += LD::ld(hcount + slot * kBuckets + i);
             int b2 = bi + 1;
-            while (b2 < kBuckets - 1 && hcount[slot * kBuckets + b2] == 0u) b2++;
-            if (b2 < kBuckets - 1 && upto + hcount[slot * kBuckets + b2] < tots[0]) bi = b2;
+            while (b2 < kBuckets - 1 && LD::ld(hcount + slot * kBuckets + b2) == 0u) b2++;
+            if (b2 < kBuckets - 1 && upto + LD::ld(hcount + slot * kBuckets + b2) < tots[0]) bi = b2;
         }
         s_split = bi;
     }
@@ -502,7 +518,7 @@
             ch.buf = 1 - nd.buf;
             ch.slot = -1; ch.child0 = -1; ch.nchild = 0;
             ch.klin = nd.klin; ch.kquad = nd.kquad;
-            ch.psplit = split | (nd.degenerate ? 0x10000 : 0);
+            ch.psplit = split | ((degenerate < 0 ? nd.degenerate : degenerate) ? 0x10000 : 0);
             double s0[NQ], s1[NQ];
 #pragma unroll
             for (int q = 0; q < NQ; q++) {
@@ -518,6 +534,13 @@
     }
     for (int i = b; i < 2 * kNodeResetElems; i += kBuckets)
         node_reset_element(nodes[nd.child0 + i / kNodeResetElems], i % kNodeResetElems);
+}
+template <bool W>
+__global__ __launch_bounds__(512) void k_cut(NodeDev *nodes, const int *__restrict__ round_nodes, const double *__restrict__ hist,
+                                             const unsigned long long *__restrict__ hsize, const unsigned int *__restrict__ hcount,
+                                             unsigned char *lut, const int fault, const RoundDyn *__restrict__ dyn) {
+    if (dyn && (int)blockIdx.x >= dyn->nr) return;
+    cut_node<W, LdPlain>(nodes, nodes[round_nodes[blockIdx.x]], hist, hsize, hcount, lut, fault, -1);
 }
 
 __global__ __launch_bounds__(256) void k_count(QuantBuffers qb, const Tile *__restrict__ tiles, const NodeDev *__restrict__ nodes,
@@ -710,11 +733,11 @@
     }
 }
 
-template <bool W, bool INV>
+template <bool W, bool INV, bool FOLD>
 __global__ __launch_bounds__(256, (W || INV) ? 2 : 3) void k_scatter_bin(QuantBuffers qb, const Tile *__restrict__ tiles, int ntiles, NodeDev *nodes,
                                                                         const NodeDev *__restrict__ nodes_ro,
                                                                         const unsigned long long *__restrict__ tileoff, const int from_end,
-                                                                        const RoundDyn *__restrict__ dyn) {
+                                                                        const RoundDyn *__restrict__ dyn, const RoundFold fold) {
     constexpr int R = kTileP / 256;
     static_assert(R * 4 == 32, "one 32-lane group per child");
     __shared__ unsigned int wcnt[2][2][R * 4];
@@ -768,7 +791,9 @@
         classify(t, b0, nodes_ro[t.node].split, 0, cr);
         baseL = lane64(toff, 0); baseR = lane64(toff, 32);
     }
+    unsigned run = 0;
     for (int ti = tfirst; ti < tlast; ti++) {
+        run++;
         const int par = (ti - tfirst) & 1;
         const NodeDev &nd = nodes_ro[t.node];
         const int child0 = nd.child0;
@@ -851,6 +876,21 @@
                         if (a[14 * side + 2 * i + 1] != 0.0) unsafeAtomicAdd(&chn.acc[blockIdx.x & (kSlots - 1)][i][1], a[14 * side + 2 * i + 1]);
                     }
                 }
+            }
+            if constexpr (FOLD) {
+                if (wid == 0) {
+                    const int r = nd.slot;
+                    int last = 0;
+                    if (lane == 0) {
+                        const LqCtl *c = fold.ctl;
+                        last = node_ticket(&fold.ctl->ticket[1][r], run, (unsigned)(c->tP0[r + 1] - c->tP0[r])) ? 1 : 0;
+                    }
+                    if (__builtin_amdgcn_readfirstlane(last)) {
+                        lq_child_moments<LdAgent>(nodes, fold.ctl, child0, 2 * r, false);
+                        lq_child_moments<LdAgent>(nodes, fold.ctl, child0 + 1, 2 * r + 1, false);
+                    }
+                }
+                run = 0;
             }
         }
         if (more) {
@@ -956,14 +996,25 @@
 template <bool W, bool GQ>
 static void launch_hist_t(const QuantBuffers &qb, const Tile *d_tiles, int ntiles, size_t px, NodeDev *d_nodes, double *d_hist,
                           unsigned long long *d_hsize, unsigned int *d_hcount, hipStream_t s, bool from_end,
-                          const RoundDyn *dyn = nullptr, const double *px_src = nullptr) {
+                          const RoundDyn *dyn = nullptr, const double *px_src = nullptr, const RoundFold *fold = nullptr) {
     constexpr int NQ = GQ ? (W ? 14 : 10) : (W ? 4 : 3);
     size_t lds = (size_t)NQ * 2 * kBuckets * sizeof(double) + kBuckets * (sizeof(unsigned int) + sizeof(unsigned long long));
     static PerDeviceOnce attr_set;
-    if (attr_set.first()) HIP_CHECK(hipFuncSetAttribute((const void *)k_hist<W, GQ>, hipFuncAttributeMaxDynamicSharedMemorySize, (int)lds));
+    if (attr_set.first()) {
+        HIP_CHECK(hipFuncSetAttribute((const void *)k_hist<W, GQ, false>, hipFuncAttributeMaxDynamicSharedMemorySize, (int)lds));
+        if constexpr (!GQ) HIP_CHECK(hipFuncSetAttribute((const void *)k_hist<W, false, true>, hipFuncAttributeMaxDynamicSharedMemorySize, (int)lds));
+    }
     KTIME_DYN(GQ ? "k_hist_gq" : "k_hist_lq", s, (W ? 34.0 : 26.0), px, px_src);
     const int g = std::min(ntiles, 256 * (GQ ? 1 : 4));
-    hipLaunchKernelGGL((k_hist<W, GQ>), g, 512, lds, s, qb, d_tiles, ntiles, d_nodes, d_hist, d_hsize, d_hcount, from_end ? 1 : 0, dyn);
+    if constexpr (!GQ) {
+        if (dyn && fold) {
+            const int fault = g_debug_fault.load(std::memory_order_relaxed);
+            hipLaunchKernelGGL((k_hist<W, false, true>), g, 512, lds, s, qb, d_tiles, ntiles, d_nodes, d_hist, d_hsize, d_hcount, from_end ? 1 : 0, dyn, *fold, fault);
+            HIP_CHECK(hipGetLastError());
+            return;
+        }
+    }
+    hipLaunchKernelGGL((k_hist<W, GQ, false>), g, 512, lds, s, qb, d_tiles, ntiles, d_nodes, d_hist, d_hsize, d_hcount, from_end ? 1 : 0, dyn, RoundFold{}, 0);
     HIP_CHECK(hipGetLastError());
 }
 
@@ -1039,7 +1090,7 @@
 
 void launch_hist(const QuantBuffers &qb, bool gq, const Tile *d_tiles, int ntiles, size_t px, NodeDev *d_nodes,
                  double *d_hist, unsigned long long *d_hsize, unsigned int *d_hcount, hipStream_t s, bool from_end, bool fixed_point,
-                 const RoundDyn *dyn, const double *px_src) {
+                 const RoundDyn *dyn, const double *px_src, const RoundFold *fold) {
     if (!ntiles) return;
     if (gq && fixed_point) {
         if (qb.weighted) launch_hist_fix<true>(qb, d_tiles, ntiles, px, d_nodes, d_hist, d_hsize, d_hcount, s, from_end);
@@ -1047,9 +1098,9 @@
         return;
     }
     if (qb.weighted) { if (gq) launch_hist_t<true, true>(qb, d_tiles, ntiles, px, d_nodes, d_hist, d_hsize, d_hcount, s, from_end);
-                       else launch_hist_t<true, false>(qb, d_tiles, ntiles, px, d_nodes, d_hist, d_hsize, d_hcount, s, from_end, dyn, px_src); }
+                       else launch_hist_t<true, false>(qb, d_tiles, ntiles, px, d_nodes, d_hist, d_hsize, d_hcount, s, from_end, dyn, px_src, fold); }
     else { if (gq) launch_hist_t<false, true>(qb, d_tiles, ntiles, px, d_nodes, d_hist, d_hsize, d_hcount, s, from_end);
-           else launch_hist_t<false, false>(qb, d_tiles, ntiles, px, d_nodes, d_hist, d_hsize, d_hcount, s, from_end, dyn, px_src); }
+           else launch_hist_t<false, false>(qb, d_tiles, ntiles, px, d_nodes, d_hist, d_hsize, d_hcount, s, from_end, dyn, px_src, fold); }
 }
 
 std::atomic<int> g_debug_fault{0};
@@ -1066,7 +1117,7 @@
 void launch_partition(const QuantBuffers &qb, const Tile *d_ptiles, int nptiles, size_t px, const int *d_round_nodes,
                       const int *d_node_tile0, int nround, NodeDev *d_nodes, const unsigned char *d_lut,
                       unsigned int *d_tilecnt, unsigned long long *d_tileoff, bool fuse_cov, hipStream_t s, bool invariant, bool from_end,
-                      const RoundDyn *dyn, const double *px_src, bool gated) {
+                      const RoundDyn *dyn, const double *px_src, bool gated, const RoundFold *fold) {
     const int fe = (from_end ? 1 : 0) | (gated ? 2 : 0);
     if (!nround) return;
     if (nptiles) { KTIME_DYN("k_count", s, 2.0, px, px_src); hipLaunchKernelGGL(k_count, nptiles, 256, 0, s, qb, d_ptiles, d_nodes, d_lut, d_tilecnt, fe & 1, dyn); }
@@ -1076,11 +1127,18 @@
         KTIME_DYN(fuse_cov ? "k_scatter_cov" : "k_scatter", s, (qb.weighted ? 66.0 : 50.0), px, px_src);
         if (fuse_cov) {
             const int gb = std::min(nptiles, 256 * ((invariant || qb.weighted) ? 2 : 3));
-            if (invariant) {
-                if (qb.weighted) hipLaunchKernelGGL((k_scatter_bin<true, true>), gb, 256, 0, s, qb, d_ptiles, nptiles, d_nodes, (const NodeDev *)d_nodes, d_tileoff, fe, dyn);
-                else hipLaunchKernelGGL((k_scatter_bin<false, true>), gb, 256, 0, s, qb, d_ptiles, nptiles, d_nodes, (const NodeDev *)d_nodes, d_tileoff, fe, dyn);
-            } else if (qb.weighted) hipLaunchKernelGGL((k_scatter_bin<true, false>), gb, 256, 0, s, qb, d_ptiles, nptiles, d_nodes, (const NodeDev *)d_nodes, d_tileoff, fe, dyn);
-            else hipLaunchKernelGGL((k_scatter_bin<false, false>), gb, 256, 0, s, qb, d_ptiles, nptiles, d_nodes, (const NodeDev *)d_nodes, d_tileoff, fe, dyn);
+            const RoundFold nf{};
+            if (dyn && fold) {
+                if (invariant) {
+                    if (qb.weighted) hipLaunchKernelGGL((k_scatter_bin<true, true, true>), gb, 256, 0, s, qb, d_ptiles, nptiles, d_nodes, (const NodeDev *)d_nodes, d_tileoff, fe, dyn, *fold);
+                    else hipLaunchKernelGGL((k_scatter_bin<false, true, true>), gb, 256, 0, s, qb, d_ptiles, nptiles, d_nodes, (const NodeDev *)d_nodes, d_tileoff, fe, dyn, *fold);
+                } else if (qb.weighted) hipLaunchKernelGGL((k_scatter_bin<true, false, true>), gb, 256, 0, s, qb, d_ptiles, nptiles, d_nodes, (const NodeDev *)d_nodes, d_tileoff, fe, dyn, *fold);
+                else hipLaunchKernelGGL((k_scatter_bin<false, false, true>), gb, 256, 0, s, qb, d_ptiles, nptiles, d_nodes, (const NodeDev *)d_nodes, d_tileoff, fe, dyn, *fold);
+            } else if (invariant) {
+                if (qb.weighted) hipLaunchKernelGGL((k_scatter_bin<true, true, false>), gb, 256, 0, s, qb, d_ptiles, nptiles, d_nodes, (const NodeDev *)d_nodes, d_tileoff, fe, dyn, nf);
+                else hipLaunchKernelGGL((k_scatter_bin<false, true, false>), gb, 256, 0, s, qb, d_ptiles, nptiles, d_nodes, (const NodeDev *)d_nodes, d_tileoff, fe, dyn, nf);
+            } else if (qb.weighted) hipLaunchKernelGGL((k_scatter_bin<true, false, false>), gb, 256, 0, s, qb, d_ptiles, nptiles, d_nodes, (const NodeDev *)d_nodes, d_tileoff, fe, dyn, nf);
+            else hipLaunchKernelGGL((k_scatter_bin<false, false, false>), gb, 256, 0, s, qb, d_ptiles, nptiles, d_nodes, (const NodeDev *)d_nodes, d_tileoff, fe, dyn, nf);
             if (gated) {
                 HIP_CHECK(hipGetLastError());
                 const int fg = (from_end ? 1 : 0) | 4;
```

Result: slower. 3165 (-1.4%).
